# olofson/audiality2

Measured on AMD Instinct MI355X. Metric: voice-samples/sec + max realtime voices @48kHz, higher is better.
Workload: dtype int32; 1 GPU; 65536 voices 2xwtosc->panmix, 256 per group voice inline->fbdelay->fbdelay (benchmark/fmtest4.a2s delay settings; 256 groups, 512 fbdelays), 48 kHz, fragment=64, stereo (BASELINE configs[3]); voices_per_gpu=65536, chain=osc2-pan, groups=256

## Files before the change

### audiality2_amd/build.py

```python
import hashlib
import os
import shutil
import subprocess

HERE = os.path.dirname(os.path.abspath(__file__))
ROOT = os.path.dirname(HERE)
HIPCC = shutil.which("hipcc") or "/opt/rocm/bin/hipcc"


MARK = b"A2AMD_SRCHASH:"


def source_hash(sources, cmd=()):
    h = hashlib.sha256()
    for s in sources:
        h.update(os.path.basename(s).encode() + b"\0")
        with open(s, "rb") as f:
            h.update(f.read())
        h.update(b"\0")
    h.update(" ".join(cmd).encode())
    return h.hexdigest()[:32]


def stamped_hash(lib, mark=MARK):
    if not os.path.exists(lib):
        return None
    with open(lib, "rb") as f:
        blob = f.read()
    i = blob.find(mark)
    if i < 0:
        return None
    return blob[i + len(mark):i + len(mark) + 32].decode("ascii", "replace")


ENGMARK = b"A2AMD_ENGHASH:"


def engine_hash(engine):
    files = []
    for d in ("include", "src", os.path.join("src", "units"), os.path.join("src", "drivers")):
        p = os.path.join(engine, d)
        if os.path.isdir(p):
            files += [os.path.join(p, f) for f in sorted(os.listdir(p)) if f.endswith((".h", ".h.cmake", ".h.in"))]
    return source_hash(files, (stamped_hash(os.path.join(HERE, "liba2amd_units.so")) or "",))


def _stale(target, want):
    return stamped_hash(target) != want


def _define(h):
    return '-DA2AMD_SRCHASH="%s"' % h


def build_lib(force=False):
    csrc = os.path.join(HERE, "csrc")
    srcs = [os.path.join(csrc, f) for f in ("a2amd_host.cpp", "a2amd_sched.cpp", "a2amd_render.cpp", "a2amd_dist.cpp",
                                            "a2amd_vm.cpp", "a2amd_kernels.hip", "a2amd_fast.hip", "a2amd_vm.hip", "a2amd_wavecap.hip", "a2amd_wavepost.hip", "a2amd_win.hip", "a2amd_vmwin.hip", "a2amd_noise.hip", "a2amd_noisepan.hip", "a2amd_noisefiltpan.hip", "a2amd_cutsweep.hip", "a2amd_oscbare.hip")]
    deps = srcs + [os.path.join(csrc, "a2amd_host.h"), os.path.join(csrc, "a2amd_switches.h"), os.path.join(csrc, "a2amd_device.h"), os.path.join(csrc, "a2amd_dsp.h"),
                   os.path.join(csrc, "a2amd_fm.h"), os.path.join(csrc, "a2amd_vmcore.h"), os.path.join(csrc, "a2amd_taps.h"), os.path.join(csrc, "a2amd_winctl.h"), os.path.join(csrc, "a2amd_vmdev.h"), os.path.join(csrc, "a2amd_noisemap.h"), os.path.join(csrc, "a2amd_noisevoice.h"), os.path.join(csrc, "a2amd_settled.h"), os.path.join(csrc, "a2amd_cutsweep.h"), os.path.join(csrc, "a2amd_filt.h"), os.path.join(ROOT, "include", "a2amd.h"),
                   os.path.join(ROOT, "include", "a2amd_noise.h"), os.path.join(ROOT, "include", "a2amd_noisepan.h"), os.path.join(ROOT, "include", "a2amd_noisefilt.h"), os.path.join(ROOT, "include", "a2amd_sweep.h"), os.path.join(ROOT, "include", "a2amd_wavepost.h"),
                   os.path.join(ROOT, "include", "a2amd_bus.h"), os.path.join(ROOT, "include", "a2amd_oscbare.h"), os.path.join(ROOT, "include", "a2amd_fbdpan.h"), os.path.join(ROOT, "include", "a2amd_buswin.h"), os.path.join(ROOT, "include", "a2amd_vmbatch.h"), os.path.join(ROOT, "include", "a2amd_vm.h")]
    out = os.path.join(HERE, "liba2amd.so")
    flags = ["--offload-arch=gfx950", "-O3", "-std=c++17", "-fPIC", "-shared", "-Wno-unused-value"]
    want = source_hash(deps, flags)
    if force or _stale(out, want):
        subprocess.run([HIPCC] + flags + [_define(want), "-o", out] + srcs, check=True)
    return out


def build_units(force=False):
    src = os.path.join(HERE, "csrc", "a2amd_units.c")
    deps = [src, os.path.join(ROOT, "include", "a2amd.h"), os.path.join(ROOT, "include", "a2amd_noise.h"), os.path.join(ROOT, "include", "a2amd_noisepan.h"),
            os.path.join(ROOT, "include", "a2amd_noisefilt.h"), os.path.join(ROOT, "include", "a2amd_sweep.h"), os.path.join(ROOT, "include", "a2amd_bus.h"),
            os.path.join(ROOT, "include", "a2amd_wavepost.h"), os.path.join(ROOT, "include", "a2amd_oscbare.h"), os.path.join(ROOT, "include", "a2amd_fbdpan.h"), os.path.join(ROOT, "include", "a2amd_buswin.h"), os.path.join(ROOT, "include", "a2amd_vmbatch.h"), os.path.join(ROOT, "include", "a2amd_plugin.h"),
            os.path.join(ROOT, "include", "a2amd_walk.h"), os.path.join(ROOT, "include", "a2amd_vm.h")]
    out = os.path.join(HERE, "liba2amd_units.so")
    flags = ["-O2", "-Wall", "-fPIC", "-shared"]
    want = source_hash(deps, flags)
    if force or _stale(out, want):
        subprocess.run(["gcc"] + flags + [_define(want), "-o", out, src,
                        "-L" + HERE, "-la2amd", "-ldl", "-lpthread", "-lm", "-Wl,-rpath,$ORIGIN"], check=True)
    return out


def build_walk(force=False, engine=None):
    engine = engine or os.environ.get("A2_ENGINE_SRC", "/root/reference")
    out = os.path.join(HERE, "liba2amd_walk.so")
    src = os.path.join(HERE, "csrc", "a2amd_walk.c")
    own = [src, os.path.join(ROOT, "include", "a2amd_walk.h"), os.path.join(ROOT, "include", "a2amd_vm.h"),
           os.path.join(ROOT, "include", "a2amd_plugin.h")]
    flags = ["-O2", "-Wall", "-fPIC", "-shared"]
    want = source_hash(own, flags)
    kept = os.path.join(ROOT, "oracle", "_ref", "liba2amd_walk.so")
    if not (os.path.exists(os.path.join(engine, "src", "internals.h")) and shutil.which("cmake")):
        if (not os.path.exists(out) or _stale(out, want)) and not _stale(kept, want):
            shutil.copyfile(kept, out)
        if os.path.exists(out) and _stale(out, want):
            raise RuntimeError(f"{out} was not built from this tree's a2amd_walk.c (stamp {stamped_hash(out)}, "
                               f"sources {want}) and the engine's source tree ({engine}) is not here to rebuild it")
        return out if os.path.exists(out) else None
    inc = os.path.join(HERE, "_engine_include")
    weng = engine_hash(engine)
    if force or _stale(out, want) or stamped_hash(out, ENGMARK) != weng:
        subprocess.run(["cmake", f"-DENGINE={engine}", f"-DOUT={inc}", "-P", os.path.join(HERE, "csrc", "engine_header.cmake")],
                       check=True, stdout=subprocess.DEVNULL)
        subprocess.run(["gcc"] + flags + [_define(want), '-DA2AMD_ENGHASH="%s"' % weng, "-I" + inc] +
                       ["-I" + os.path.join(engine, d) for d in ("include", "src", "src/units", "src/drivers")] +
                       ["-o", out, src, "-L" + HERE, "-la2amd_units", "-la2amd", "-ldl", "-lpthread", "-Wl,-rpath,$ORIGIN"],
                       check=True)
    if stamped_hash(kept) != want or stamped_hash(kept, ENGMARK) != weng:
        os.makedirs(os.path.dirname(kept), exist_ok=True)
        shutil.copyfile(out, kept)
    return out


def build_oracle(force=False):
    odir = os.path.join(ROOT, "oracle")
    targets = ["restate"]
    if os.path.exists("/root/reference/src/core.c") and shutil.which("cmake"):
        targets += ["ref", "tools", "optionb"]
    subprocess.run(["make", "-s", "-C", odir] + (["-B"] if force else []) + targets, check=True)
    return os.path.join(odir, "liba2oracle.so")


def build_all(force=False):
    lib = build_lib(force)
    build_units(force)
    build_walk(force)
    return lib, build_oracle(force)
```

### audiality2_amd/csrc/a2amd_device.h

```cpp
#pragma once
#include <stdint.h>

#define A2D_MAXCHAIN   16
#define A2D_CHAIN_INLINE 8
#define A2D_MAXBATCH 256
#define FBW_MAXWIN (2 * A2D_MAXBATCH)
#define A2D_USTATE    24
#define A2D_MAXCH      8
#define A2D_FRAG      64
#define A2D_MIPS      10
#define A2D_FBD_BUFSIZE 131072
#define A2D_MAXPHINC  512
#define A2D_COEF_WORDS 3
#define A2D_WTOSC_MAXLENGTH (0x01000000 - 1 - 131)

enum { A2D_WTOSC = 0, A2D_PANMIX, A2D_FILTER12, A2D_FBDELAY, A2D_INLINE, A2D_XINSERT,
	A2D_FM1, A2D_FM2, A2D_FM3, A2D_FM4, A2D_FM3P, A2D_FM4P, A2D_FM2R, A2D_FM4R,
	A2D_DC, A2D_WAVESHAPER, A2D_DCBLOCK, A2D_LIMITER, A2D_XSINK, A2D_XSOURCE };
#define A2D_IS_FM(k) ((k) >= A2D_FM1 && (k) <= A2D_FM4R)

enum { A2D_OSC_OFF = 0, A2D_OSC_NOISE, A2D_OSC_WAVE, A2D_OSC_MIPWAVE };

#define A2D_DESC(kind, add, nin, nout, wired) \
	(((uint32_t)(kind) << 24) | ((uint32_t)(add) << 4) | ((uint32_t)(nin) << 8) | \
	 ((uint32_t)(nout) << 12) | ((uint32_t)(wired) << 16))
#define A2D_KIND(d)  ((d) >> 24)
#define A2D_ADD(d)   (((d) >> 4) & 1u)
#define A2D_NIN(d)   (((d) >> 8) & 15u)
#define A2D_NOUT(d)  (((d) >> 12) & 15u)
#define A2D_WIRED(d) (((d) >> 16) & 1u)

enum {
	OW_MODE = 0, OW_WAVE, OW_DPHASE, OW_PHASE_LO, OW_PHASE_HI, OW_NOISE,
	OW_PRAMPING, OW_P = 7, OW_A = 11, OW_SEED = 15 };
enum {
	PW_VOL = 0, PW_PAN = 4 };
enum {
	FW_Q = 0, FW_LP = 4, FW_BP, FW_HP, FW_F1, FW_D1A, FW_D1B, FW_D2A, FW_D2B,
	FW_F1NEXT, FW_RAMP };
enum {
	DW_FBDELAY = 0, DW_LDELAY, DW_RDELAY, DW_DRYGAIN, DW_FBGAIN, DW_LGAIN,
	DW_RGAIN, DW_BUFPOS, DW_BUFIDX };

enum {
	CW_VALUE = 0, CW_MODE = 4 };
enum {
	SW_AMOUNT = 0 };
enum {
	BW_F1 = 0, BW_D1A, BW_D1B, BW_D2A, BW_D2B };
enum {
	LW_RELEASE = 0, LW_THRESHOLD, LW_PEAK };
enum {
	MW_SLOT = 0 };
enum {
	FO_A = 0, FO_FB = 4, FO_P = 8, FO_LASTPITCH = 12, FO_PHASE, FO_DPHASE, FO_LAST, FO_WORDS };
#define A2D_FMSTATE 64

#define A2D_WF_RAWTAPS 0x40000000u

struct A2DWave {
	int32_t  type;
	uint32_t flags;
	uint32_t period;
	uint32_t size[A2D_MIPS];
	uint32_t off[A2D_MIPS];
	uint32_t pad;
};

struct A2DVoice {
	int32_t nunits;
	int32_t unit[A2D_CHAIN_INLINE];
	int32_t out_off, out_nch;
	int32_t own_off, own_nch;
	int32_t pad[3];
};

static_assert(sizeof(A2DVoice) == 64, "the voice record is one 64-byte line");
struct A2DVoiceExt { int32_t unit[A2D_MAXCHAIN - A2D_CHAIN_INLINE]; };

struct A2DRec {
	uint32_t head;
	int32_t  value;
	uint32_t dur;
	uint32_t start;
};
enum { R_SEG = 1, R_WRITE, R_INIT, R_KILL, R_F1SET, R_F1RAMP, R_NOISESEED, R_NOP };
#define A2D_HEAD(frag, op, unit, reg) \
	((uint32_t)(frag) | ((uint32_t)(op) << 16) | ((uint32_t)(unit) << 24) | ((uint32_t)(reg) << 28))
#define A2D_RFRAG(h) ((h) & 0xffffu)
#define A2D_ROP(h)   (((h) >> 16) & 0xffu)
#define A2D_RUNIT(h) (((h) >> 24) & 15u)
#define A2D_RREG(h)  (((h) >> 28) & 15u)

struct A2DRun { int32_t first, count; };

#define A2D_VM_NOWRITE 0xffu
#define A2D_VM_TRAPWRITE 0xfeu
#define A2D_VM_MAXCUT  2
#define A2D_VM_MAXENV  2
#define A2D_VM_MAXPOS  8
#define A2D_VM_ENVPOS  14
#define A2D_ENV_LUTSHIFT 6
#define A2D_ENV_LUTSIZE  (1 << A2D_ENV_LUTSHIFT)
#define A2D_ENV_LUTS     8
struct A2DVmEnv {
	int32_t ramper[4];
	int32_t lut;
	int32_t scale, offset, out;
	int32_t active;
	uint8_t regbase;
	uint8_t k;
	uint8_t target;
	uint8_t pad;
};
struct A2DVmVoice {
	uint32_t waketime;
	uint32_t code, ncode;
	uint16_t pc;
	uint8_t  state, ncut;
	int32_t  voice;
	int32_t  fault;
	uint8_t  cmap[64];
	uint8_t  kind[A2D_MAXCHAIN];
	uint8_t  cutpos[A2D_VM_MAXCUT];
	uint8_t  pad[2];
	int32_t  cut[A2D_VM_MAXCUT][4];
	A2DVmEnv env[A2D_VM_MAXENV];
	int32_t  nenv;
	uint32_t exit_when;
	int32_t  has_exit;
	int32_t  r[64];
};

struct A2DVmParams {
	A2DVmVoice     *vmv;
	const int      *list;
	int32_t         n;
	const uint32_t *code;
	const uint32_t *ptab;
	const int32_t  *f1tab;
	const uint16_t *envlut;
	A2DRun         *runs;
	A2DRun         *vmrun;
	A2DRec         *recs;
	uint32_t        rec_base, rec_cap;
	uint32_t       *total;
	uint32_t        now;
	uint32_t        msdur;
	int32_t         samplerate, basepitch;
	int32_t         nfrags;
	uint8_t         fragframes[A2D_MAXBATCH];
	uint8_t         fragbase[A2D_MAXBATCH];
};

enum { XW_SLOT = 0, XW_MODE = 1 };
#define A2D_XIO_HALF ((size_t)A2D_MAXBATCH * 8 * A2D_FRAG)
#define A2D_XIO_SLOT (2 * A2D_XIO_HALF)

#define A2D_FAST_FCH 8
#define A2D_OSC2_FCH 4
#define A2D_MAXVPW   32

struct A2DParams {
	const A2DVoice *voices;
	const A2DVoiceExt *vext;
	const uint32_t *udesc;
	int32_t        *ustate;
	int32_t        *vactive;
	const A2DRun   *runs;
	const A2DRec   *recs;
	const A2DWave  *waves;
	const int16_t  *wavepool;
	const int32_t  *wavecoef;
	int32_t        *busmem;
	int32_t        *fbdmem;
	const uint32_t *ptab;
	int32_t        *fmstate;
	const uint32_t *fmsine;
	int32_t *xio;
	const uint32_t *nseed;
	const int32_t  *nslot;
	int32_t         nnoise;
	const int32_t  *cutf;
	const int32_t  *cslot;
	int32_t         ncut;
	int32_t         nfrags;
	int32_t         samplerate;
	int32_t         debug;
	uint8_t         fragframes[A2D_MAXBATCH];
	uint16_t        fragstart[A2D_MAXBATCH];
};

#ifdef __HIPCC__
static inline __host__ __device__ bool a2d_noise_seed(const A2DParams &p, int f, int ui, unsigned *seed)
{
	if(!p.nseed)
		return false;
	const int k = p.nslot[ui];
	if(k <= 0 || k > p.nnoise)
		return false;
	*seed = p.nseed[(size_t)f * (size_t)p.nnoise + (size_t)(k - 1)];
	return true;
}
#endif

#ifdef __HIPCC__
static inline __host__ __device__ bool a2d_cut_coeff(const A2DParams &p, int f, int ui, int *f1)
{
	if(p.ncut <= 0)
		return false;
#if defined(__HIP_DEVICE_COMPILE__)
	typedef const __attribute__((address_space(4))) A2DParams *CP;
	typedef const __attribute__((address_space(4))) int32_t *CI;
	uintptr_t qa = (uintptr_t)&p;
	asm volatile("" : "+s"(qa));
	const CP q = (CP)qa;
	const int ncut = q->ncut;
	const int k = *((CI)(uintptr_t)q->cslot + ui);
	if(k <= 0 || k > ncut)
		return false;
	const int v = *((CI)(uintptr_t)q->cutf + ((size_t)f * (size_t)ncut + (size_t)(k - 1)));
#else
	const int k = p.cslot[ui];
	if(k <= 0 || k > p.ncut)
		return false;
	const int v = p.cutf[(size_t)f * (size_t)p.ncut + (size_t)(k - 1)];
#endif
	if(v < 0)
		return false;
	*f1 = v;
	return true;
}
#endif

struct A2DCutSweep { int32_t ramper[4]; int32_t unit, slot, pad[2]; };
int a2d_launch_cut_sweep(const A2DCutSweep *list, int n, int f0, int count, unsigned frames, int32_t *cutf, int stride,
		size_t words, int32_t *cslot, int nunits, void *stream);
int a2d_launch_cut_resolve(int32_t *cutf, size_t words, const int32_t *f1tab, void *stream);

struct A2DNoiseOsc { uint32_t ph_lo, ph_hi, dphase; int32_t unit, slot, pad[3]; };
int a2d_launch_noise_seeds(const A2DNoiseOsc *osc, int n, uint32_t start, int f0, int count, unsigned frames,
		uint32_t *seed, int stride, size_t seed_words, int32_t *nslot, int nunits, void *stream);

int a2d_launch_leaf_noisepan(const A2DParams *dparams, const A2DParams &hp, const int *dlist, int nlist, int vpw, void *stream);
int a2d_launch_leaf_noisefiltpan(const A2DParams *dparams, const A2DParams &hp, const int *dlist, int nlist, int vpg, void *stream);
int a2d_launch_leaf_oscbare(const A2DParams *dparams, const A2DParams &hp, const int *dlist, int nlist, int vpw, void *stream);

int a2d_launch_vm(const A2DVmParams &vp, int emit, void *stream);
int a2d_launch_vm_pool(const A2DVmParams &vp, unsigned *out, void *stream);
#define A2D_WIN_STAGED 2
struct A2DVmwOut {
	A2DVmVoice *vmv;
	int        *ustate;
	int        *vactive;
	A2DRun     *runs;
	uint32_t   *total;
	uint32_t   *idle;
};
int a2d_launch_vm_commit(const A2DVmParams &vp, const A2DParams &hp, int nosc, int filt, const A2DVmwOut &from, void *stream);
int a2d_launch_vm_win(const A2DVmParams &vp, const A2DParams &hp, int nosc, int filt, int fa, int fb, uint32_t now_fa,
		uint32_t batch_end, int *wslot, int *wext, int *wscr, unsigned *widx, unsigned *wtop, unsigned wcap, void *stream,
		const A2DVmwOut *out = nullptr);
#define A2D_VMW_ROW (64 - 1 - 1)

int a2d_launch_voices(const A2DParams *dparams, const int *dlist, int nlist, int vpw, void *stream);
enum { A2D_STAGED_NONE = 0, A2D_STAGED_PHASES, A2D_STAGED_FULL };
struct A2DCommit { const int *list; int nlist, nosc; const int *ustage; const unsigned char *staged; };
struct A2DCommitSet { A2DCommit c[2]; int n; };
int a2d_launch_leaf_oscpan(const A2DParams *dparams, const A2DParams &hp, const int *dlist, int nlist,
		int vpw, int ysplit, int *ustage, unsigned char *staged, void *stream, void *event_after_main, A2DCommit *defer);
int a2d_launch_bus_driver(const A2DParams *dparams, const int *dlist, int nlist, int nfrags, int consume,
		const A2DCommitSet *commits, void *stream, int *master_host = nullptr, int ramping = 0);
int a2d_launch_commit(const A2DParams &hp, const A2DCommit &cm, void *stream);
int a2d_launch_bus_fbdchain(const A2DParams *dparams, const int *dlist, int nlist, int consume, void *stream);
int a2d_launch_bus_fbdpan(const A2DParams *dparams, const int *dlist, int nlist, int consume, void *stream, int windows = 0);
int a2d_launch_park(int32_t *stage, int32_t *bus, unsigned words, void *stream);
int a2d_launch_add_bus(int32_t *dst, int32_t *src, unsigned words, void *stream);
int a2d_launch_add_inject(const int32_t *inj, int32_t *bus, int nch, int n, int nfrags, void *stream);
int a2d_launch_build_coef(const int16_t *pool, int *coef, unsigned lo, unsigned hi, void *stream);
int a2d_launch_capture(const int32_t *bus, int32_t *dst, const uint32_t *fragpos, int nfrags, int nch, void *stream);
int a2d_launch_wave_from_pcm(const int32_t *pcm, int16_t *pool, const uint32_t *off, const uint32_t *size, int levels, int looped,
		int pre, int post, void *stream);
int a2d_launch_wave_level0(const int32_t *pcm, int16_t *d, unsigned size, void *stream);
int a2d_launch_wave_finish(int16_t *pool, const uint32_t *off, const uint32_t *size, int levels, int looped, int pre, int post,
		void *stream);
unsigned a2d_wavepost_scratch_words(unsigned size, unsigned flags, unsigned chunk);
int a2d_launch_wave_level0_post(const int32_t *pcm, int16_t *d, unsigned size, unsigned flags, unsigned chunk, uint32_t *scratch,
		void *stream);
int a2d_osc2filtpan_max_vpg(void);
int a2d_launch_leaf_osc2filtpan(const A2DParams *dparams, const A2DParams &hp, const int *dlist, int nlist,
		int vpg, void *stream);
int a2d_launch_leaf_oscfiltpan(const A2DParams *dparams, const A2DParams &hp, const int *dlist, int nlist,
		int vpw, void *stream);
int a2d_launch_scatter_runs(const int *didx, const A2DRun *dval, int n, A2DRun *druns, void *stream);
int a2d_launch_leaf_osc2pan(const A2DParams *dparams, const A2DParams &hp, const int *dlist, int nlist,
		int vpw, int ysplit, int *ustage, unsigned char *staged, void *stream, A2DCommit *defer);
struct A2Switches;
int a2d_launch_leaf_recs(const A2Switches &sw, const A2DParams *dparams, const A2DParams &hp, int nosc, int filt, const int *dlist,
		int nlist, int vpw, void *stream, int skip_empty = 0);
#define A2D_WIN_WORDS 24
#define A2D_WIN_SLOTWORDS(nosc, filt) ((filt) ? ((nosc) == 1 ? 20 : 24) : ((nosc) == 1 ? 12 : 20))
int a2d_launch_win_ctl(const A2DParams *dparams, const A2DParams &hp, int nosc, int filt, const int *dlist, int nlist,
		int skip_empty, int fa, int fb, int *wslot, int *wext, unsigned *widx, unsigned *wtop, unsigned wcap, int *wrc,
		void *stream);
int a2d_launch_win_render(const A2Switches &sw, const A2DParams &hp, int nosc, int filt, const int *dlist, int nlist, int fa, int fb,
		const int *wslot, const int *wext, const unsigned *widx, void *stream);
int a2d_launch_leaf_recs_all(const A2Switches &sw, const A2DParams *dparams, const A2DParams &hp, const int *const *lists, const int *counts,
		int vpw, void *stream, int skip_mask = 0);
int a2d_launch_leaf_fmpan(const A2DParams *dparams, const A2DParams &hp, int kind, const int *dlist, int nlist,
		int vpw, void *stream);
int a2d_launch_leaf_fmpan_all(const A2DParams *dparams, const A2DParams &hp, const int *dlist,
		const int *count8, int vpw, void *stream);
```

### audiality2_amd/csrc/a2amd_fast.hip

```cpp
#include <hip/hip_runtime.h>
#include <type_traits>
#include <algorithm>
#include <stdlib.h>
#include "a2amd_device.h"
#include "a2amd_switches.h"
#include "a2amd_dsp.h"
#include "a2amd_fm.h"
#include "a2amd_filt.h"

#include "a2amd_taps.h"

__global__ void k_build_coef(const int16_t *__restrict__ pool, int *__restrict__ coef, unsigned lo, unsigned hi)
{
	const unsigned j = lo + blockIdx.x * blockDim.x + threadIdx.x;
	if(j >= hi)
		return;
	const int dm = pool[j - 1], d0 = pool[j], d1 = pool[j + 1], d2 = pool[j + 2];
	const int c = (d1 - dm) >> 1;
	const int a = (3 * (d0 - d1) + d2 - dm) >> 1;
	const int b = dm - d0 + c - a;
	int *e = coef + A2D_COEF_WORDS * (size_t)j;
	e[0] = a;
	e[1] = b;
	e[2] = (int)(((unsigned)c << 16) | ((unsigned)d0 & 0xffffu));
// ... 398 lines not shown
					phs[j] = ph;
					ph += (uint64_t)dph * (unsigned)nfr[j];
				}
			}
			const unsigned ldph = lane_dph(lane, dph);
			const int cb = coef_base(doff);
			if((raw_mask >> v) & 1ull) {
				const int16_t *d = wavepool + doff;
#pragma unroll
				for(int h = 0; h < FAST_FCH; h += 4) {
					Quad16 qa[4], qb[4];
					unsigned pa[4], pb[4];
#pragma unroll
					for(int j = 0; j < 4; ++j) {
						pa[j] = tap_phase(phs[h + j], ldph);
						pb[j] = pa[j] + (dph16 >> 1);
						qa[j] = *(const Quad16 *)(d + (int)(pa[j] >> 8) - 1);
						qb[j] = *(const Quad16 *)(d + (int)(pb[j] >> 8) - 1);
					}
#pragma unroll
					for(int j = 0; j < 4; ++j) {
						int sm = inter_quads(qa[j], qb[j], pa[j], pb[j]);
						int x = mul64s(sm, amp, 17);
						x = (lane < nfr[h + j]) ? x : 0;
						acc0[h + j] = wadd(acc0[h + j], mul64s(x, v0, 24));
						acc1[h + j] = wadd(acc1[h + j], mul64s(x, v1, 24));
					}
				}
			} else
#pragma unroll
			for(int h = 0; h < FAST_FCH; h += 4) {
				Coef4 ka[4], kb[4];
				unsigned pa[4], pb[4];
#pragma unroll
				for(int j = 0; j < 4; ++j) {
					pa[j] = tap_phase(phs[h + j], ldph);
					asm("" : "+v"(pa[j]));
					pb[j] = pa[j] + (dph16 >> 1);
					ka[j] = coef_at(crs, cb, pa[j]);
					kb[j] = coef_at(crs, cb, pb[j]);
				}
#pragma unroll
				for(int j = 0; j < 4; ++j) {
					int sm = inter_coefs(ka[j], pa[j], kb[j], pb[j]);
					int x = mul64s(sm, amp, 17);
					x = (lane < nfr[h + j]) ? x : 0;
					acc0[h + j] = wadd(acc0[h + j], mul64s(x, v0, 24));
					acc1[h + j] = wadd(acc1[h + j], mul64s(x, v1, 24));
				}
			}
			if(last_slice && c == c_hi - 1) {
				const bool me = lane == v;
				const uint64_t endph = ph << (unsigned)rdl(dv[DV_MM], v);
				WRL(phlo_l, (int)(unsigned)endph);
				WRL(phhi_l, (int)(unsigned)(endph >> 32));
			}
		}
		flush_acc(busmem, cur_off, cur_nch, f0, nf, lane, dbg, acc0, acc1);
	}

	const unsigned long long todo_mask = unsettled_mask & __ballot(lane % nslices == slice);
	if(todo_mask) {
		for(int f0 = 0; f0 < nfrags; f0 += FAST_FCH) {
			const int nf = min((int)FAST_FCH, nfrags - f0);
			int acc0[FAST_FCH], acc1[FAST_FCH];
#pragma unroll
			for(int j = 0; j < FAST_FCH; ++j)
				acc0[j] = acc1[j] = 0;
			int cur_off = rdl(my_off, 0), cur_nch = rdl(my_nch, 0);
			for(int v = 0; v < nv; ++v) {
				if(!((todo_mask >> v) & 1ull))
					continue;
				const int voff = rdl(my_off, v);
				if(voff != cur_off) {
					flush_acc(busmem, cur_off, cur_nch, f0, nf, lane, dbg, acc0, acc1);
					cur_off = voff;
					cur_nch = rdl(my_nch, v);
				}
				OscS o;
				Ramp vol, pan;
				const int *src = f0 ? ustage : ustate;
				osc_from_mem(o, src + (size_t)rdl(u0, v) * A2D_USTATE);
				{
					const volatile int *wpv = src + (size_t)rdl(u1, v) * A2D_USTATE;
					vol.value = rfl(wpv[0]); vol.target = rfl(wpv[1]); vol.delta = rfl(wpv[2]); vol.timer = rfl(wpv[3]);
					pan.value = rfl(wpv[4]); pan.target = rfl(wpv[5]); pan.delta = rfl(wpv[6]); pan.timer = rfl(wpv[7]);
				}
				for(int j = 0; j < nf; ++j) {
					int o0 = 0, o1 = 0;
					oscpan_fragment(g, o, vol, pan, frames_of(ffr, f0 + j), lane, o0, o1);
#pragma unroll
					for(int jj = 0; jj < FAST_FCH; ++jj)
						if(jj == j) {
							acc0[jj] = wadd(acc0[jj], o0);
							acc1[jj] = wadd(acc1[jj], o1);
						}
				}
				if(lane == 0) {
					osc_to_mem(ustage + (size_t)rdl(u0, v) * A2D_USTATE, o);
					int *wpv = ustage + (size_t)rdl(u1, v) * A2D_USTATE;
					wpv[0] = vol.value; wpv[1] = vol.target; wpv[2] = vol.delta; wpv[3] = vol.timer;
					wpv[4] = pan.value; wpv[5] = pan.target; wpv[6] = pan.delta; wpv[7] = pan.timer;
				}
			}
			flush_acc(busmem, cur_off, cur_nch, f0, nf, lane, dbg, acc0, acc1);
			__builtin_amdgcn_fence(__ATOMIC_RELEASE, "wavefront");
			__builtin_amdgcn_s_waitcnt(0);
		}
	}

	if(mine && dv[DV_SETTLED] && last_slice) {
		int *w0 = ustage + (size_t)u0 * A2D_USTATE;
		w0[OW_PHASE_LO] = phlo_l;
		w0[OW_PHASE_HI] = phhi_l;
	}
	if(ustage != ustate && lane < nv)
		stage_mark(staged + first + lane, mine, dv[DV_SETTLED] != 0, last_slice, lane % nslices == slice);
}

DEV void commit_block(const A2DCommit &cm, int block, const A2DVoice *__restrict__ voices, int *__restrict__ ustate)
{
	const int i = block * 256 + threadIdx.x;
	if(i >= cm.nlist * cm.nosc)
		return;
	const int e = i / cm.nosc, o = i - e * cm.nosc;
	const int what = cm.staged[e];
	if(what == A2D_STAGED_NONE)
		return;
	const A2DVoice &vc = voices[cm.list[e]];
	const size_t a = (size_t)vc.unit[o] * A2D_USTATE;
	ustate[a + OW_PHASE_LO] = cm.ustage[a + OW_PHASE_LO];
	ustate[a + OW_PHASE_HI] = cm.ustage[a + OW_PHASE_HI];
	if(what != A2D_STAGED_FULL)
		return;
	for(int k = 0; k < 15; ++k)
		if(k != OW_NOISE && k != OW_PHASE_LO && k != OW_PHASE_HI)
			ustate[a + k] = cm.ustage[a + k];
	if(o == 0) {
		const size_t ap = (size_t)vc.unit[cm.nosc] * A2D_USTATE;
		for(int k = 0; k < 8; ++k)
			ustate[ap + k] = cm.ustage[ap + k];
	}
}

DEV int commit_blocks(const A2DCommit &cm) { return (cm.nlist * cm.nosc + 255) / 256; }

__global__ __launch_bounds__(256)
void k_commit_oscpan(A2DCommit cm, const A2DVoice *__restrict__ voices, int *__restrict__ ustate)
{
	commit_block(cm, blockIdx.x, voices, ustate);
}

#define OSC2_FCH A2D_OSC2_FCH
enum { OV_MODE = 0, OV_WAVE, OV_DPHASE, OV_PHLO, OV_PHHI, OV_PRAMP, OV_P = 6, OV_A = 10, OV_NWORDS = 14 };
enum { OD_MM = 0, OD_DPH, OD_SIZEM, OD_DOFF, OD_NWORDS };

DEV void osc_from_lanes(OscS &o, const int (&so)[OV_NWORDS], int v)
{
	o.mode = rdl(so[OV_MODE], v);
	o.wave = rdl(so[OV_WAVE], v);
	o.dphase = (unsigned)rdl(so[OV_DPHASE], v);
	o.phase = (uint64_t)(unsigned)rdl(so[OV_PHLO], v) | ((uint64_t)(unsigned)rdl(so[OV_PHHI], v) << 32);
	o.p_ramping = rdl(so[OV_PRAMP], v);
	o.p.value = rdl(so[OV_P], v); o.p.target = rdl(so[OV_P + 1], v);
	o.p.delta = rdl(so[OV_P + 2], v); o.p.timer = rdl(so[OV_P + 3], v);
	o.a.value = rdl(so[OV_A], v); o.a.target = rdl(so[OV_A + 1], v);
	o.a.delta = rdl(so[OV_A + 2], v); o.a.timer = rdl(so[OV_A + 3], v);
	o.noise = 0;
	o.seed = 0;
}

DEV void osc_to_lanes(int (&so)[OV_NWORDS], const OscS &o, bool me)
{
	WRL(so[OV_MODE], o.mode);
	WRL(so[OV_WAVE], o.wave);
	WRL(so[OV_DPHASE], (int)o.dphase);
	WRL(so[OV_PHLO], (int)(unsigned)o.phase);
	WRL(so[OV_PHHI], (int)(unsigned)(o.phase >> 32));
	WRL(so[OV_PRAMP], o.p_ramping);
	WRL(so[OV_P], o.p.value); WRL(so[OV_P + 1], o.p.target);
	WRL(so[OV_P + 2], o.p.delta); WRL(so[OV_P + 3], o.p.timer);
	WRL(so[OV_A], o.a.value); WRL(so[OV_A + 1], o.a.target);
	WRL(so[OV_A + 2], o.a.delta); WRL(so[OV_A + 3], o.a.timer);
}

#define OSC2_WPE 4
__global__ __launch_bounds__(64 * FAST_WPB) __attribute__((amdgpu_waves_per_eu(OSC2_WPE, OSC2_WPE)))
void k_leaf_osc2pan(const A2DParams *__restrict__ pp, const int *__restrict__ list, int nlist, int vpw,
		int ysplit, const A2DVoice *__restrict__ voices, const int *ustate, int *ustage,
		const int16_t *__restrict__ wavepool, const A2DWave *__restrict__ waves,
		const uint32_t *__restrict__ ptab, int *__restrict__ busmem, const int *__restrict__ wavecoef,
		unsigned char *__restrict__ staged)
{
	const A2DParams &p = *pp;
	const int wv = rfl((int)(threadIdx.x >> 6));
	const int lane = threadIdx.x & 63;
	const int first = (blockIdx.x * FAST_WPB + wv) * vpw;
	if(first >= nlist)
		return;
	const int nv = min(vpw, nlist - first);
	const int nfrags = p.nfrags;
	const int dbg = p.debug;
	FastPtrs g = { wavepool, waves, ptab, dbg };
	const CoefRsrc crs = coef_rsrc(wavecoef);

	const int nchunks = (nfrags + OSC2_FCH - 1) / OSC2_FCH;
	const int per = (nchunks + ysplit - 1) / ysplit;
	const int slice = blockIdx.y;
	const int c_lo = slice * per, c_hi = min(nchunks, c_lo + per);
	const bool last_slice = c_hi >= nchunks;
	if(c_lo >= nchunks)
		return;
	const int nslices = (nchunks + per - 1) / per;

	int ffr[A2D_MAXBATCH / 64], fst[A2D_MAXBATCH / 64];
#pragma unroll
	for(int k = 0; k < A2D_MAXBATCH / 64; ++k) {
		ffr[k] = (k * 64 + lane < nfrags) ? p.fragframes[k * 64 + lane] : 0;
		fst[k] = (k * 64 + lane < nfrags) ? p.fragstart[k * 64 + lane] : 0;
	}

	int od[2][OD_NWORDS], amp_l[2] = { 0, 0 }, phlo_l[2] = { 0, 0 }, phhi_l[2] = { 0, 0 };
	int v0l = 0, v1l = 0, settled_l = 0;
	int uu[3] = { 0, 0, 0 }, my_off = -1, my_nch = 2;
	bool mine = false;
#pragma unroll
	for(int o = 0; o < 2; ++o)
#pragma unroll
		for(int k = 0; k < OD_NWORDS; ++k)
			od[o][k] = 0;
	if(lane < nv)
		mine = p.runs[list[first + lane]].count == 0;
	if(mine) {
		const A2DVoice &vc = voices[list[first + lane]];
		my_off = vc.out_off;
		my_nch = vc.out_nch;
		bool settled = true;
		int wave_l[2], dphase_l[2];
#pragma unroll
		for(int o = 0; o < 2; ++o) {
			uu[o] = vc.unit[o];
			const int *w = ustate + (size_t)uu[o] * A2D_USTATE;
			wave_l[o] = w[OW_WAVE];
			dphase_l[o] = w[OW_DPHASE];
			amp_l[o] = w[OW_A];
			phlo_l[o] = w[OW_PHASE_LO];
			phhi_l[o] = w[OW_PHASE_HI];
			settled = settled && a2s_osc_settled(w[OW_MODE], (unsigned)dphase_l[o], w[OW_PRAMPING], w + OW_P, w + OW_A);
		}
		uu[2] = vc.unit[2];
		const int *wp = ustate + (size_t)uu[2] * A2D_USTATE;
		int sp[8];
#pragma unroll
		for(int k = 0; k < 8; ++k)
			sp[k] = wp[k];
		settled = settled && a2s_arrived(sp + PW_VOL, sp + PW_PAN);
		if(settled) {
#pragma unroll
			for(int o = 0; o < 2; ++o)
				settled = settled_wave(waves + wave_l[o], (unsigned)dphase_l[o], od[o], settled);
			a2s_pan_gains(sp[PW_VOL], sp[PW_PAN], a2s_pan_over(sp[PW_PAN]), &v0l, &v1l);
		}
		settled_l = settled ? 1 : 0;
	}
	const unsigned long long unsettled_mask = __ballot(mine && !settled_l);

	for(int c = c_lo; c < c_hi; ++c) {
		const int f0 = c * OSC2_FCH;
		const int nf = min((int)OSC2_FCH, nfrags - f0);
		int acc0[OSC2_FCH], acc1[OSC2_FCH], nfr[OSC2_FCH];
#pragma unroll
		for(int j = 0; j < OSC2_FCH; ++j) {
			acc0[j] = acc1[j] = 0;
			nfr[j] = (j < nf) ? frames_of(ffr, f0 + j) : 0;
		}
		const unsigned before = (unsigned)frames_of(fst, f0);
		unsigned pre[OSC2_FCH];
		pre[0] = 0;
#pragma unroll
		for(int j = 1; j < OSC2_FCH; ++j)
			pre[j] = pre[j - 1] + (unsigned)nfr[j - 1];
		int cur_off = rdl(my_off, 0), cur_nch = rdl(my_nch, 0);
		for(int v = 0; v < nv; ++v) {
			if(!rdl(settled_l, v))
				continue;
			const int voff = rdl(my_off, v);
			if(voff != cur_off) {
				flush_acc(busmem, cur_off, cur_nch, f0, nf, lane, dbg, acc0, acc1);
				cur_off = voff;
				cur_nch = rdl(my_nch, v);
			}
			const int v0 = rdl(v0l, v), v1 = rdl(v1l, v);
			int xs[OSC2_FCH];
			uint64_t endph[2];
			Coef4 ka[2][OSC2_FCH], kb[2][OSC2_FCH];
			unsigned pa[2][OSC2_FCH], pb[2][OSC2_FCH];
			int amps[2];
#pragma unroll
			for(int o = 0; o < 2; ++o) {
				const unsigned mm = (unsigned)rdl(od[o][OD_MM], v), dph = (unsigned)rdl(od[o][OD_DPH], v);
				const unsigned sizem = (unsigned)rdl(od[o][OD_SIZEM], v), doff = (unsigned)rdl(od[o][OD_DOFF], v);
				amps[o] = rdl(amp_l[o], v);
				const uint64_t phase = (uint64_t)(unsigned)rdl(phlo_l[o], v) |
						((uint64_t)(unsigned)rdl(phhi_l[o], v) << 32);
				uint64_t ph = (phase >> mm) + (uint64_t)before * dph;
				const unsigned ldph = lane_dph(lane, dph);
				const int cb = coef_base(doff);
				uint64_t phs[OSC2_FCH];
				if(!(sizem & (sizem - 1)) && !(ph >> 48)) {
					const uint64_t mask = ((uint64_t)sizem << 24) - 1;
#pragma unroll
					for(int j = 0; j < OSC2_FCH; ++j)
						phs[j] = (ph + (uint64_t)dph * pre[j]) & mask;
					ph = phs[OSC2_FCH - 1] + (uint64_t)dph * (unsigned)nfr[OSC2_FCH - 1];
				} else {
#pragma unroll
					for(int j = 0; j < OSC2_FCH; ++j) {
						ph = wrap_phase(ph, sizem);
						phs[j] = ph;
						ph += (uint64_t)dph * (unsigned)nfr[j];
					}
				}
#pragma unroll
				for(int j = 0; j < OSC2_FCH; ++j) {
					pa[o][j] = tap_phase(phs[j], ldph);
					asm("" : "+v"(pa[o][j]));
					pb[o][j] = pa[o][j] + (dph >> 17);
					ka[o][j] = coef_at(crs, cb, pa[o][j]);
					kb[o][j] = coef_at(crs, cb, pb[o][j]);
				}
				endph[o] = ph << mm;
			}
#pragma unroll
			for(int o = 0; o < 2; ++o)
#pragma unroll
				for(int j = 0; j < OSC2_FCH; ++j) {
					const int y = mul64s(inter_coefs(ka[o][j], pa[o][j], kb[o][j], pb[o][j]), amps[o], 17);
					xs[j] = o ? wadd(xs[j], y) : y;
				}
#pragma unroll
			for(int j = 0; j < OSC2_FCH; ++j) {
				const int x = (lane < nfr[j]) ? xs[j] : 0;
				acc0[j] = wadd(acc0[j], mul64s(x, v0, 24));
				acc1[j] = wadd(acc1[j], mul64s(x, v1, 24));
			}
			if(last_slice && c == c_hi - 1) {
				const bool me = lane == v;
#pragma unroll
				for(int o = 0; o < 2; ++o) {
					WRL(phlo_l[o], (int)(unsigned)endph[o]);
					WRL(phhi_l[o], (int)(unsigned)(endph[o] >> 32));
				}
			}
		}
		flush_acc(busmem, cur_off, cur_nch, f0, nf, lane, dbg, acc0, acc1);
	}

	const unsigned long long todo_mask = unsettled_mask & __ballot(lane % nslices == slice);
	if(todo_mask) {
		for(int f0 = 0; f0 < nfrags; f0 += OSC2_FCH) {
			const int nf = min((int)OSC2_FCH, nfrags - f0);
			int acc0[OSC2_FCH], acc1[OSC2_FCH];
#pragma unroll
			for(int j = 0; j < OSC2_FCH; ++j)
				acc0[j] = acc1[j] = 0;
			int cur_off = rdl(my_off, 0), cur_nch = rdl(my_nch, 0);
			for(int v = 0; v < nv; ++v) {
				if(!((todo_mask >> v) & 1ull))
					continue;
				const int voff = rdl(my_off, v);
				if(voff != cur_off) {
					flush_acc(busmem, cur_off, cur_nch, f0, nf, lane, dbg, acc0, acc1);
					cur_off = voff;
					cur_nch = rdl(my_nch, v);
				}
				OscS oa, ob;
				Ramp vol, pan;
				const int *src = f0 ? ustage : ustate;
				osc_from_mem(oa, src + (size_t)rdl(uu[0], v) * A2D_USTATE);
				osc_from_mem(ob, src + (size_t)rdl(uu[1], v) * A2D_USTATE);
				{
					const volatile int *wpv = src + (size_t)rdl(uu[2], v) * A2D_USTATE;
					vol.value = rfl(wpv[0]); vol.target = rfl(wpv[1]); vol.delta = rfl(wpv[2]); vol.timer = rfl(wpv[3]);
					pan.value = rfl(wpv[4]); pan.target = rfl(wpv[5]); pan.delta = rfl(wpv[6]); pan.timer = rfl(wpv[7]);
				}
				for(int j = 0; j < nf; ++j) {
					const int n = frames_of(ffr, f0 + j);
					int o0 = 0, o1 = 0;
					const OscPend pa_ = osc_fragment_begin(g, oa, n, lane), pb_ = osc_fragment_begin(g, ob, n, lane);
					const int x = wadd(osc_fragment_end(pa_), osc_fragment_end(pb_));
					pan_fragment_s(vol, pan, x, n, lane, o0, o1);
#pragma unroll
					for(int jj = 0; jj < OSC2_FCH; ++jj)
						if(jj == j) {
							acc0[jj] = wadd(acc0[jj], o0);
							acc1[jj] = wadd(acc1[jj], o1);
						}
				}
				if(lane == 0) {
					osc_to_mem(ustage + (size_t)rdl(uu[0], v) * A2D_USTATE, oa);
					osc_to_mem(ustage + (size_t)rdl(uu[1], v) * A2D_USTATE, ob);
					int *wpv = ustage + (size_t)rdl(uu[2], v) * A2D_USTATE;
					wpv[0] = vol.value; wpv[1] = vol.target; wpv[2] = vol.delta; wpv[3] = vol.timer;
					wpv[4] = pan.value; wpv[5] = pan.target; wpv[6] = pan.delta; wpv[7] = pan.timer;
				}
			}
			flush_acc(busmem, cur_off, cur_nch, f0, nf, lane, dbg, acc0, acc1);
			__builtin_amdgcn_fence(__ATOMIC_RELEASE, "wavefront");
			__builtin_amdgcn_s_waitcnt(0);
		}
	}

	if(mine && settled_l && last_slice) {
#pragma unroll
		for(int o = 0; o < 2; ++o) {
			int *w = ustage + (size_t)uu[o] * A2D_USTATE;
			w[OW_PHASE_LO] = phlo_l[o];
			w[OW_PHASE_HI] = phhi_l[o];
		}
	}
	if(ustage != ustate && lane < nv)
		stage_mark(staged + first + lane, mine, settled_l != 0, last_slice, lane % nslices == slice);
}

#define RECS_FCH 4
#define RECS_WPB 8

DEV void osc_init_s(const FastPtrs &g, OscS &o, int pitch)
{
	o.wave = -1;
	o.mode = A2D_OSC_OFF;
	o.phase = 0;
	o.p_ramping = 0;
	o.noise = 0;
	o.seed = 0;
	ramp_init(o.a, 0);
	ramp_init(o.p, pitch);
	o.dphase = (unsigned)rfl((int)p2i(g.ptab, o.p.value >> 8));
}

DEV void osc_write_s(const FastPtrs &g, OscS &o, int reg, int v, int start, int dur)
{
	switch(reg) {
	  case 0: {
		int wt = 0;
		o.wave = v;
		if(v >= 0) {
			const A2DWave *w = g.waves + v;
			wt = w->type;
			if(wt == 3 && w->size[0] > (unsigned)A2D_WTOSC_MAXLENGTH)
				wt = 0;
		}
		if(wt == 3)
			o.mode = A2D_OSC_MIPWAVE;
		else if(wt == 1)
			o.mode = A2D_OSC_NOISE;
		else {
			o.wave = -1;
			o.mode = A2D_OSC_OFF;
		}
		break;
	  }
	  case 1:
		ramp_set(o.p, v, start, dur);
		if(!dur)
			o.p_ramping = 1;
		break;
	  case 2:
		ramp_set(o.a, v, start, dur);
		break;
	  case 3:
		if(o.wave < 0)
			o.phase = 0;
		else {
			const unsigned period = g.waves[o.wave].period;
			const int ph = (int)((unsigned)v + ((((unsigned)start) * (o.dphase >> 8)) >> 8));
			o.phase = (uint64_t)(((int64_t)ph * (int64_t)period) * 256);
		}
		break;
	}
}

enum { FS_Q = 0, FS_LP = 4, FS_BP, FS_HP, FS_F1, FS_D1, FS_D2, FS_F1NEXT, FS_RAMP, FS_NWORDS };
struct FiltS { Ramp q; int lp, bp, hp, f1, d1, d2, f1next, ramp; };

extern "C" __device__ int a2d_writelane(int src, int lane, int old) __asm("llvm.amdgcn.writelane.i32");
DEV int writelane_s(int y, int val, int sel)
{
	return a2d_writelane(val, sel, y);
}

#define F12_JSTEP \
	"s_nop 1\n\t" \
	"v_mov_b32_dpp %[bsh], %[B] wave_shr:1 row_mask:0xf bank_mask:0xf\n\t" \
	"v_ashrrev_i32 %[ds], 4, %[bsh]\n\t" \
	"v_mul_lo_u32 %[t1], %[F], %[ds]\n\t" \
	"v_ashrrev_i32 %[t1], 8, %[t1]\n\t" \
	"v_mul_lo_u32 %[t2], %[Q], %[ds]\n\t" \
	"v_ashrrev_i32 %[t2], 8, %[t2]\n\t" \
	"v_add_u32_dpp %[L], %[L], %[t1] wave_shr:1 row_mask:0xf bank_mask:0xf\n\t" \
	"v_sub_u32 %[H], %[X], %[L]\n\t" \
	"v_sub_u32 %[H], %[H], %[t2]\n\t" \
	"v_ashrrev_i32 %[t1], 4, %[H]\n\t" \
	"v_mul_lo_u32 %[t1], %[F], %[t1]\n\t" \
	"v_ashrrev_i32 %[t1], 8, %[t1]\n\t" \
	"v_add_u32 %[B], %[t1], %[bsh]\n\t"
DEV int filt_window_j(FiltS &fs, int x, int off, int len, int lane)
{
// ... 1640 lines not shown
#pragma unroll
	for(int k = 0; k < FBC_MAXD; ++k)
		if(k < nd) {
			const int *w = p.ustate + (size_t)vc.unit[k + 1] * A2D_USTATE;
			d[k].fb = rfl(w[DW_FBDELAY]); d[k].l = rfl(w[DW_LDELAY]); d[k].r = rfl(w[DW_RDELAY]);
			d[k].dry = rfl(w[DW_DRYGAIN]); d[k].fbg = rfl(w[DW_FBGAIN]); d[k].lg = rfl(w[DW_LGAIN]); d[k].rg = rfl(w[DW_RGAIN]);
			d[k].pos = rfl(w[DW_BUFPOS]);
			d[k].b0 = p.fbdmem + (size_t)rfl(w[DW_BUFIDX]) * 2 * A2D_FBD_BUFSIZE;
			d[k].b1 = d[k].b0 + A2D_FBD_BUFSIZE;
			d[k].add = rfl((int)A2D_ADD(p.udesc[vc.unit[k + 1]]));
			dmin = min(dmin, min(d[k].fb, min(d[k].l, d[k].r)));
			dmax = max(dmax, max(d[k].fb, max(d[k].l, d[k].r)));
		}
	__syncthreads();
	const bool rest = at_rest != 0;
	int rv0 = 0, rv1 = 0;
	if(rest) {
		const int vk = fr[0][0], vp = mul64s(fr[0][2], vk, 24);
		rv0 = wsub(vk, vp); rv1 = wadd(vk, vp);
		if(fr[0][4]) {
			const int lim = wshl(vk, 1);
			if(rv0 > lim) rv0 = lim;
			if(rv1 > lim) rv1 = lim;
		}
	}
	const int rf = max(1, min(dmin, A2D_FBD_BUFSIZE - dmax) / A2D_FRAG);
	int *own = p.busmem + vc.own_off;
	int *out = p.busmem + vc.out_off;
	const int out_nch = vc.out_nch;
	for(int f0 = 0; f0 < nfrags; f0 += rf) {
		const int fend = min(nfrags, f0 + rf);
		for(int idx = f0 * A2D_FRAG + (int)threadIdx.x; idx < fend * A2D_FRAG; idx += FBC_THREADS) {
			const int f = idx >> 6, lane = idx & 63;
			if(lane >= p.fragframes[f])
				continue;
			const int t = (int)p.fragstart[f] + lane;
			int *src = own + (size_t)f * 2 * A2D_FRAG;
			int x0 = src[lane], x1 = src[A2D_FRAG + lane];
			if(consume) {
				src[lane] = 0;
				src[A2D_FRAG + lane] = 0;
			}
#pragma unroll
			for(int k = 0; k < FBC_MAXD; ++k)
				if(k < nd) {
					const FbdU &u = d[k];
					const int pos = wadd(u.pos, t);
					int o0 = mul64s(u.b1[(pos - u.fb) & M], u.fbg, 16);
					int o1 = mul64s(u.b0[(pos - u.fb) & M], u.fbg, 16);
					const int t0 = u.b0[(pos - u.l) & M], t1 = u.b1[(pos - u.r) & M];
					u.b0[pos & M] = wadd(x0, o0);
					u.b1[pos & M] = wadd(x1, o1);
					o0 = wadd(o0, mul64s(t0, u.lg, 16));
					o1 = wadd(o1, mul64s(t1, u.rg, 16));
					o0 = wadd(o0, mul64s(x0, u.dry, 16));
					o1 = wadd(o1, mul64s(x1, u.dry, 16));
					if(u.add) {
						x0 = wadd(x0, o0);
						x1 = wadd(x1, o1);
					} else {
						x0 = o0;
						x1 = o1;
					}
				}
			int v0 = rv0, v1 = rv1;
			if(!rest) {
				int r = f, wk = lane;
				if constexpr(WIN) {
					r = min((int)wfirst[f], FBW_MAXWIN - 1);
					const int rl = min((int)wfirst[f + 1], FBW_MAXWIN) - 1;
					while(r < rl && lane >= (fr[r][4] >> 16))
						++r;
					wk = lane - ((fr[r][4] >> 8) & 0xff);
				}
				const int vk = wadd(fr[r][0], wmul(fr[r][1], wk));
				const int pk = wadd(fr[r][2], wmul(fr[r][3], wk));
				const int vp = mul64s(pk, vk, 24);
				v0 = wsub(vk, vp); v1 = wadd(vk, vp);
				if(WIN ? fr[r][4] & 1 : fr[r][4]) {
					const int lim = wshl(vk, 1);
					if(v0 > lim) v0 = lim;
					if(v1 > lim) v1 = lim;
				}
			}
			const int o0 = mul64s(x0, v0, 24), o1 = mul64s(x1, v1, 24);
			int *dst = out + (size_t)f * out_nch * A2D_FRAG;
			if(o0)
				atomicAdd(&dst[lane], o0);
			if(o1)
				atomicAdd(&dst[A2D_FRAG + lane], o1);
		}
		if(fend < nfrags)
			__syncthreads();
	}
	if(threadIdx.x == 0) {
		int total = 0;
		for(int f = 0; f < nfrags; ++f)
			total += p.fragframes[f];
#pragma unroll
		for(int k = 0; k < FBC_MAXD; ++k)
			if(k < nd)
				p.ustate[(size_t)vc.unit[k + 1] * A2D_USTATE + DW_BUFPOS] = wadd(d[k].pos, total);
	}
}

__global__ __launch_bounds__(FBC_THREADS)
void k_bus_fbdpan(const A2DParams *__restrict__ pp, const int *__restrict__ list, int nlist, int consume)
{
	bus_fbdpan<false>(pp, list, consume);
}

__global__ __launch_bounds__(FBC_THREADS)
void k_bus_fbdpan_win(const A2DParams *__restrict__ pp, const int *__restrict__ list, int nlist, int consume)
{
	bus_fbdpan<true>(pp, list, consume);
}

int a2d_launch_bus_fbdpan(const A2DParams *dparams, const int *dlist, int nlist, int consume, void *stream, int windows)
{
	if(nlist <= 0)
		return 0;
	hipLaunchKernelGGL(windows ? k_bus_fbdpan_win : k_bus_fbdpan, dim3(nlist), dim3(FBC_THREADS), 0, (hipStream_t)stream,
			dparams, dlist, nlist, consume);
	return (int)hipGetLastError();
}

int a2d_launch_leaf_oscpan(const A2DParams *dparams, const A2DParams &hp, const int *dlist, int nlist,
		int vpw, int ysplit, int *ustage, unsigned char *staged, void *stream, void *event_after_main, A2DCommit *defer)
{
	if(nlist <= 0)
		return 0;
	vpw = vpw < 1 ? 1 : (vpw > 64 ? 64 : vpw);
	if(ysplit < 1 || !ustage || !staged)
		ysplit = 1;
	int nwaves = (nlist + vpw - 1) / vpw;
	int nblocks = (nwaves + FAST_WPB - 1) / FAST_WPB;
	hipLaunchKernelGGL(k_leaf_oscpan, dim3(nblocks, ysplit), dim3(64 * FAST_WPB), 0, (hipStream_t)stream,
			dparams, dlist, nlist, vpw, ysplit, hp.voices, (const int *)hp.ustate,
			ysplit > 1 ? ustage : hp.ustate, hp.wavepool, hp.waves, hp.ptab, hp.busmem, hp.wavecoef, staged);
	if(event_after_main)
		hipEventRecord((hipEvent_t)event_after_main, (hipStream_t)stream);
	if(ysplit > 1) {
		A2DCommit cm = { dlist, nlist, 1, ustage, staged };
		if(defer)
			*defer = cm;
		else
			a2d_launch_commit(hp, cm, stream);
	} else if(defer)
		defer->nlist = 0;
	return (int)hipGetLastError();
}

int a2d_launch_leaf_osc2pan(const A2DParams *dparams, const A2DParams &hp, const int *dlist, int nlist,
		int vpw, int ysplit, int *ustage, unsigned char *staged, void *stream, A2DCommit *defer)
{
	if(nlist <= 0)
		return 0;
	vpw = vpw < 1 ? 1 : (vpw > 64 ? 64 : vpw);
	if(ysplit < 1 || !ustage || !staged)
		ysplit = 1;
	int nwaves = (nlist + vpw - 1) / vpw;
	int nblocks = (nwaves + FAST_WPB - 1) / FAST_WPB;
	hipLaunchKernelGGL(k_leaf_osc2pan, dim3(nblocks, ysplit), dim3(64 * FAST_WPB), 0, (hipStream_t)stream,
			dparams, dlist, nlist, vpw, ysplit, hp.voices, (const int *)hp.ustate,
			ysplit > 1 ? ustage : hp.ustate, hp.wavepool, hp.waves, hp.ptab, hp.busmem, hp.wavecoef, staged);
	if(ysplit > 1) {
		A2DCommit cm = { dlist, nlist, 2, ustage, staged };
		if(defer)
			*defer = cm;
		else
			a2d_launch_commit(hp, cm, stream);
	} else if(defer)
		defer->nlist = 0;
	return (int)hipGetLastError();
}

__global__ void k_scatter_runs(const int *__restrict__ idx, const A2DRun *__restrict__ val, int n,
		A2DRun *__restrict__ runs)
{
	int i = blockIdx.x * blockDim.x + threadIdx.x;
	if(i < n)
		runs[idx[i]] = val[i];
}

int a2d_launch_scatter_runs(const int *didx, const A2DRun *dval, int n, A2DRun *druns, void *stream)
{
	if(n <= 0)
		return 0;
	hipLaunchKernelGGL(k_scatter_runs, dim3((n + 255) / 256), dim3(256), 0, (hipStream_t)stream,
			didx, dval, n, druns);
	return (int)hipGetLastError();
}

int a2d_launch_leaf_oscfiltpan(const A2DParams *dparams, const A2DParams &hp, const int *dlist, int nlist,
		int vpg, void *stream)
{
	if(nlist <= 0)
		return 0;
	vpg = vpg < 1 ? 1 : (vpg > FILT_MAXV ? FILT_MAXV : vpg);
	int nblocks = (nlist + vpg - 1) / vpg;
	size_t lds = (size_t)3 * vpg * FILT_PITCH * sizeof(int);
	hipLaunchKernelGGL(k_leaf_oscfiltpan, dim3(nblocks), dim3(64 * FILT_WAVES), lds, (hipStream_t)stream,
			dparams, dlist, nlist, vpg, hp.voices, hp.ustate, hp.wavepool, hp.waves, hp.ptab, hp.busmem, hp.wavecoef);
	return (int)hipGetLastError();
}

int a2d_osc2filtpan_max_vpg(void)
{
	const int nfull = FILT_WAVES - 1 - (FILT_WAVES / 4 - 1);
	const int v = nfull * (FILT2_LAUNCHV < FILT2_FASTV ? FILT2_LAUNCHV : FILT2_FASTV);
	return v > FILT_MAXV ? FILT_MAXV : v;
}

int a2d_launch_leaf_osc2filtpan(const A2DParams *dparams, const A2DParams &hp, const int *dlist, int nlist,
		int vpg, void *stream)
{
	if(nlist <= 0)
		return 0;
	vpg = vpg < 1 ? 1 : (vpg > FILT_MAXV ? FILT_MAXV : vpg);
	int nblocks = (nlist + vpg - 1) / vpg;
	size_t lds = (size_t)3 * vpg * FILT_PITCH * sizeof(int);
	hipLaunchKernelGGL(k_leaf_osc2filtpan, dim3(nblocks), dim3(64 * FILT_WAVES), lds, (hipStream_t)stream,
			dparams, dlist, nlist, vpg, hp.voices, hp.ustate, hp.wavepool, hp.waves, hp.ptab, hp.busmem, hp.wavecoef);
	return (int)hipGetLastError();
}

enum { PV_VOL = 0, PV_PAN = 4, PV_NWORDS = 8 };

DEV void pan_window_s(Ramp &vol, Ramp &pan, int x, int off, int len, int lane, int &acc0, int &acc1)
{
	const bool clamp = a2s_pan_over(pan.target) || a2s_pan_over(pan.value);
	ramp_prepare_s(vol, len);
	ramp_prepare_s(pan, len);
	const int k = lane - off;
	if(k >= 0 && k < len) {
		int vk = wadd(vol.value, wmul(vol.delta, k));
		int pk = wadd(pan.value, wmul(pan.delta, k));
		int vp = mul64s(pk, vk, 24);
		int v0 = wsub(vk, vp), v1 = wadd(vk, vp);
		if(clamp) {
			int lim = wshl(vk, 1);
			if(v0 > lim) v0 = lim;
			if(v1 > lim) v1 = lim;
		}
		acc0 = wadd(acc0, mul64s(x, v0, 24));
		acc1 = wadd(acc1, mul64s(x, v1, 24));
	}
	ramp_run(vol, len);
	ramp_run(pan, len);
}

template<int NOPS, int OSBITS, int PAR>
DEV void fmpan_body(const A2DParams &p, const int *__restrict__ list, int first, int nv, int lane,
		int *tile, const uint32_t *sine, const A2DVoice *__restrict__ voices, int *ustate,
		int *fmstate, const uint32_t *__restrict__ ptab, int *__restrict__ busmem)
{
	const int nfrags = p.nfrags;
	const int dbg = p.debug;
	const A2DRec *__restrict__ recs = p.recs;
	int ffr[A2D_MAXBATCH / 64];
#pragma unroll
	for(int k = 0; k < A2D_MAXBATCH / 64; ++k)
		ffr[k] = (k * 64 + lane < nfrags) ? p.fragframes[k * 64 + lane] : 0;

	int pv[PV_NWORDS];
#pragma unroll
	for(int k = 0; k < PV_NWORDS; ++k)
		pv[k] = 0;
	FmOp op[NOPS];
#pragma unroll
	for(int i = 0; i < NOPS; ++i) {
		op[i].a = op[i].fb = op[i].p = Ramp{ 0, 0, 0, 0 };
		op[i].last_pitch = op[i].last = 0;
		op[i].phase = op[i].dphase = 0;
	}
	unsigned step[NOPS], fix[NOPS];
#pragma unroll
	for(int i = 0; i < NOPS; ++i)
		step[i] = fix[i] = 0;
	int slot = -1, u0 = 0, u1 = 0, my_off = -1, my_nch = 2, v0 = 0, v1 = 0, settled = 0;
	int run_first = 0, run_count = 0, fmslot = -1;
	int actB = 0;
	const bool writer = lane < nv;
	if(lane < nv)
		slot = list[first + lane];
	else if(lane < 16 && !(p.debug & 4))
		slot = list[first + lane % nv];
	const bool mine = slot >= 0;
	const unsigned long long mine_mask = __ballot(mine);
	if(mine) {
		const A2DVoice &vc = voices[slot];
		u0 = vc.unit[0];
		u1 = vc.unit[1];
		my_off = vc.out_off;
		my_nch = vc.out_nch;
		const A2DRun run = p.runs[slot];
		run_first = run.first;
		run_count = run.count;
		actB = p.vactive[slot];
	}
	bool touched = mine && actB;
	if(touched) {
		fmslot = ustate[(size_t)u0 * A2D_USTATE + MW_SLOT];
		const int *fw = fmstate + (size_t)fmslot * A2D_FMSTATE;
#pragma unroll
		for(int i = 0; i < NOPS; ++i)
			fmop_load(op[i], fw + i * FO_WORDS);
		const int *w1 = ustate + (size_t)u1 * A2D_USTATE;
#pragma unroll
		for(int k = 0; k < 4; ++k) {
			pv[PV_VOL + k] = w1[PW_VOL + k];
			pv[PV_PAN + k] = w1[PW_PAN + k];
		}
		settled = !run_count && a2s_arrived(pv + PV_VOL, pv + PV_PAN);
		if(settled)
			a2s_pan_gains(pv[PV_VOL], pv[PV_PAN], a2s_pan_over(pv[PV_PAN]), &v0, &v1);
	}
	int curB = 0, curC = 0, actC = actB;
// ... 389 lines not shown
```

### audiality2_amd/csrc/a2amd_host.h

```cpp
#ifndef A2AMD_HOST_H
#define A2AMD_HOST_H
#include <hip/hip_runtime.h>
#include <rccl/rccl.h>
#include <dlfcn.h>
#include <math.h>
#include <stdarg.h>
#include <stdio.h>
#include <stdlib.h>
#include <string.h>
#include <algorithm>
#include <map>
#include <vector>
#include <future>

#include "../../include/a2amd.h"
#include "../../include/a2amd_vm.h"
#include "a2amd_device.h"
#include "a2amd_switches.h"

#ifndef M_PI
#define M_PI 3.14159265358979323846
#endif

namespace a2h {
// ... 231 lines not shown
	bool pred_valid = false;
	uint64_t pred_serial = 0;
	uint32_t pred_now = 0;
	uint32_t pred_span = 0;
	size_t pred_entries = 0;
	uint64_t pred_why[7] = { 0, 0, 0, 0, 0, 0, 0 };
	DevBuf<int> d_swin[2], d_swext[2], d_swscr;
	DevBuf<unsigned> d_swidx[2];
	int spec_set = 0;
	bool spec_launched_now = false;
	unsigned *d_swtop = nullptr;
	DevBuf<A2DVmVoice> d_vmv_sh;
	DevBuf<int> d_ustate_sh, d_vactive_sh;
	DevBuf<A2DRun> d_runs_sh;
	uint32_t *d_stotal = nullptr;
	unsigned *h_spec = nullptr;
	bool spec_valid = false;
	bool spec_use = false;
	int spec_nfrags = 0, spec_cls[3] = { 0, 0, 0 };
	uint8_t spec_ff[A2D_MAXBATCH], spec_fb[A2D_MAXBATCH];
	uint32_t cut_hint[16];
	int n_cut_hint = 0;
	size_t spec_cap = 0;
	size_t spec_demand = 0;
	uint64_t spec_launched = 0, spec_taken = 0, spec_overflows = 0;
	uint64_t spec_skip[4] = { 0, 0, 0, 0 }, spec_miss[4] = { 0, 0, 0, 0 };
	uint64_t spec_waits = 0;
	uint64_t rebuilt_at = 0;
	bool list_dirty = false;
	std::vector<std::pair<int, A2DVmVoice>> to_upload;
	uint32_t t0 = 0;
	bool t0_valid = false;
	uint32_t msdur = 0;
	uint64_t batch_time = 0;
	uint64_t replayed = 0;
	std::vector<int32_t> f1tab;
	std::future<std::vector<int32_t>> f1_future;
	uint32_t f1_future_sum = 0;
	uint32_t f1tab_sum = 0;
	bool f1tab_up = false;
	std::vector<A2DVmVoice> snap;
	std::vector<uint8_t> snap_have;
	int snap_fetches = 0;
	uint32_t rec_cap = 0;
	size_t rec_off = 0;
	a2amd_vm_stats stats = {};
	int unwalked = -1;
	DevBuf<A2DVmVoice> d_vmv;
	DevBuf<uint32_t> d_code;
	DevBuf<int> d_list;
	DevBuf<A2DRun> d_vmrun;
	int32_t *d_f1tab = nullptr;
	std::vector<uint16_t> envlut;
	uint16_t *d_envlut = nullptr;
	bool envlut_up = false;
	uint32_t *d_total = nullptr, *h_total = nullptr;
	uint32_t last_total = 0;
	a2amd_vm_batch_info last = {};
	A2DVmVoice *h_stage = nullptr;
	size_t h_stage_cap = 0;
};
}
using namespace a2h;

struct a2amd_ctx {
	a2amd_config cfg;
	char err[256];
	hipStream_t stream = nullptr;
	bool own_stream = false;
	hipEvent_t ev0 = nullptr, ev1 = nullptr, ev2 = nullptr;
	bool profiling = false;
	std::vector<hipEvent_t> ev_pool;
	size_t ev_used = 0;
	uint32_t ptab[128];

	std::vector<HUnit> units;
	std::vector<int> free_units, deferred_free_units;
	std::vector<HVoice> voices;
	std::vector<int> free_voices, deferred_free_voices;
	std::vector<HWave> waves;
	int building = -1;
	std::vector<int> stack;
	std::vector<A2DRec> up_recs;
	std::vector<int> up_idx, up_now;
	std::vector<A2DRun> up_val;
	std::vector<int> with_recs, prev_with_recs;
	std::vector<int> dirty_voices;
	long long serial_base = 0;
	bool o2f_quiet = true;
	int n_started_live = 0;
	int walked_started = 0;
	int n_noise = 0, n_cutoff_ramps = 0;
	std::vector<int> noise_order;
	long long noise_order_serial = -1, walk_serial = -2;
	struct NoiseStretch { int f0, count; unsigned frames; uint32_t start; size_t first, n; };
	std::vector<NoiseStretch> noise_st;
	std::vector<A2DNoiseOsc> noise_osc;
	int noise_slots = 0;
	DevBuf<uint32_t> d_nseed;
	DevBuf<int32_t> d_nslot;
	std::vector<int> sweeping;
	struct CutStretch { int f0, count; unsigned frames; size_t first, n; };
	std::vector<CutStretch> cut_st;
	std::vector<A2DCutSweep> cut_list;
	int cut_slots = 0;
	DevBuf<int32_t> d_cutf;
	DevBuf<int32_t> d_cslot;
	a2amd_sweep_batch_info last_sweeps = {};
	uint32_t n_cut_standin = 0;
	uint32_t n_cut_windows = 0;
	bool owners_all_driver = false;
	bool consume_ok = false;
	bool others_clean = false;
	bool root_clean = false;
	bool capturing = false;
	int n_clients = 0;
	int sub_resume = -1;
	int paused_at = 0;
	std::vector<int32_t> snap_ustate, snap_vactive;
	bool snap_valid = false;
	std::vector<uint8_t> defmap;
	bool defmap_used = false;
	bool defmap_dirty = false;
	std::vector<uint8_t> held;
	size_t n_held = 0;
	uint64_t walk_time = 0;
	unsigned prev_frames = 0;

	bool frag_open = false;
	int cur_frag = 0, nfrags = 0;
	unsigned fragframes[A2D_MAXBATCH];
	uint8_t fragbase[A2D_MAXBATCH];
	bool uploaded = false;

	std::vector<A2DVoice> mvoices;
	std::vector<A2DVoiceExt> mvext;
	bool long_chains = false;
	std::vector<uint32_t> mudesc;
	std::vector<A2DWave> mwaves;
	bool voices_dirty = true, udesc_dirty = true, waves_dirty = true, lists_dirty = true, ptab_dirty = true;
	std::vector<int> list_all;
	ListRange leaf[LEAF_N];
	int fm_kind_count[8] = { 0 };
	std::vector<DepthRange> depth_ranges;
	ListRange dyn[DYN_N];
	A2Switches sw;
	a2amd_batch_info last_batch = {};
	a2amd_noise_batch_info last_noise = {};
	uint32_t n_noise_standin = 0, n_noise_quiet = 0;
	uint32_t n_noise_filt_quiet = 0;
	a2amd_noise_filter_batch_info last_noise_filter = {};
	uint32_t n_bare_quiet = 0, n_bare_gliding = 0, n_bare_records = 0, n_mono_drivers = 0;
	a2amd_bare_batch_info last_bare = {};
	a2amd_fbdpan_batch_info last_fbdpan = {};
	a2amd_bus_windows_info last_buswin = {};
	a2amd_bus_info last_bus = {};
	uint32_t n_bus_windows_dropped = 0;

	size_t bus_stride_frames;
	size_t bus_used = 0;
	std::map<int, std::vector<int>> bus_free;
	std::vector<std::pair<int,int>> deferred_bus_free;

	int fbd_count = 0;
	std::vector<int> fbd_free, fbd_deferred_free, fbd_to_zero;
	int fm_count = 0;
	std::vector<int> fm_free, fm_deferred_free;

	std::vector<XioSlot> xio;
	std::vector<int> xio_free, xio_deferred_free;

	size_t wavepool_used = 0;
	std::vector<std::pair<size_t, size_t>> wavepool_free;
	std::vector<std::pair<size_t, size_t>> deferred_wavepool_free;
	std::vector<int> free_wave_slots, deferred_wave_slots;

	DevBuf<A2DVoice> d_voices;
	DevBuf<A2DVoiceExt> d_vext;
	DevBuf<uint32_t> d_udesc;
	DevBuf<int32_t> d_ustate;
	DevBuf<int32_t> d_ustage;
	DevBuf<int32_t> d_vactive;
	DevBuf<A2DRun> d_runs;
	DevBuf<A2DRec> d_recs;
	DevBuf<A2DWave> d_waves;
	DevBuf<int16_t> d_wavepool;
	DevBuf<int32_t> d_wavecoef;
	DevBuf<int32_t> d_busmem;
	DevBuf<int32_t> d_fbdmem;
	DevBuf<int32_t> d_fmstate;
	DevBuf<int32_t> d_xio;
	uint32_t *d_fmsine = nullptr;
	DevBuf<int> d_list;
	DevBuf<unsigned char> d_staged;
	DevBuf<int> d_scatter;
	uint32_t *d_ptab = nullptr;
	A2DParams *d_params = nullptr;
	DevBuf<char> d_blob;
	char *h_blob[2] = { nullptr, nullptr };
	size_t h_blob_cap[2] = { 0, 0 };
	hipEvent_t blob_ev[2] = { nullptr, nullptr };
	bool blob_busy[2] = { false, false };
	int blob_i = 0;
	const int *d_dyn = nullptr;
	A2DParams hparams;
	hipGraph_t graph[12] = {};
	hipGraphExec_t gexec[12] = {};
	const int32_t *gdst[12] = {};
	bool gdirect[12] = {};
	uint32_t gconsume[12] = {};
	struct Capture { int32_t *d = nullptr; size_t cap = 0, n = 0; bool on = false; uint32_t *d_fragpos = nullptr; } capture;
	DevBuf<uint32_t> d_wavepost;
	uint64_t wave_h2d_bytes = 0;
	uint32_t waves_uploaded = 0, waves_resident = 0;
	int32_t *master_dst = nullptr;
	bool master_direct = false;
	int32_t *h_master = nullptr;
	size_t h_master_cap = 0;
	bool blob_quiet = false;
	int blob_nfrags = 0;
	unsigned blob_frames[A2D_MAXBATCH];
	int quiet_streak = 0;
	struct Readback {
		int32_t *h = nullptr;
		size_t cap = 0;
		hipEvent_t ev = nullptr;
		int nfrags = 0;
		unsigned total = 0;
		uint8_t frames[A2D_MAXBATCH];
	} rb[2];
	int rb_head = 0, rb_count = 0;

	ncclComm_t comm = nullptr;
	int dist_rank = 0, dist_ranks = 1;
	bool dist_local = false;
	hipEvent_t grp_ev = nullptr;

	std::vector<int> moving;
	size_t n_moving_listed = 0;
	DevBuf<int> d_win, d_wext, d_wrc, d_wscr;
	DevBuf<unsigned> d_widx;
	unsigned *d_wtop = nullptr;
	unsigned *h_wtop = nullptr;
	hipEvent_t wtop_ev = nullptr;
	bool wtop_pending = false;
	hipStream_t win_fork[7] = { nullptr, nullptr, nullptr, nullptr, nullptr, nullptr, nullptr };
	hipEvent_t win_fev[8] = { nullptr, nullptr, nullptr, nullptr, nullptr, nullptr, nullptr, nullptr };
	hipStream_t win_stream = nullptr;
	hipEvent_t win_ev[5] = { nullptr, nullptr, nullptr, nullptr, nullptr };

	a2amd_stats stats;
	VmHost vm;

	int fail(int code, const char *fmt, ...)
	{
		va_list ap;
		va_start(ap, fmt);
		vsnprintf(err, sizeof(err), fmt, ap);
		va_end(ap);
		snprintf(g_err, sizeof(g_err), "%s", err);
		return code;
	}
};

static inline void use_device(const a2amd_ctx *c) { (void)hipSetDevice(c->cfg.device); }

namespace a2h {
template<class T>
int grow(a2amd_ctx *c, DevBuf<T> &b, size_t need, size_t elem_mult, bool keep)
{
	if(need <= b.cap)
		return 0;
	size_t ncap = std::max(need, b.cap ? b.cap * 2 : (elem_mult >= 65536 ? (size_t)2 : (size_t)1024));
	T *nd = nullptr;
	HIPCHK(c, hipMalloc((void **)&nd, ncap * elem_mult * sizeof(T)));
	if(keep && b.d && b.cap) {
		HIPCHK(c, hipStreamSynchronize(c->stream));
		HIPCHK(c, hipMemcpyAsync(nd, b.d, b.cap * elem_mult * sizeof(T), hipMemcpyDeviceToDevice, c->stream));
	}
	if(keep)
		HIPCHK(c, hipMemsetAsync((char *)nd + b.cap * elem_mult * sizeof(T), 0,
				(ncap - b.cap) * elem_mult * sizeof(T), c->stream));
	if(keep)
		HIPCHK(c, hipStreamSynchronize(c->stream));
	if(b.d) {
		HIPCHK(c, hipStreamSynchronize(c->stream));
		if(c->vm.pred_stream)
			HIPCHK(c, hipStreamSynchronize(c->vm.pred_stream));
		HIPCHK(c, hipFree(b.d));
	}
	b.d = nd;
	b.cap = ncap;
	return 0;
}

inline int rec_tag(const a2amd_ctx *c) { return c->frag_open ? c->cur_frag : c->nfrags; }
static inline bool is_held(const a2amd_ctx *c, int vi)
{
	return (size_t)vi < c->held.size() && c->held[vi];
}

static inline void unhold(a2amd_ctx *c, int vi)
{
	if(is_held(c, vi)) {
		c->held[vi] = 0;
		--c->n_held;
// ... 65 lines not shown
```

### audiality2_amd/csrc/a2amd_render.cpp

```cpp
#include "a2amd_host.h"

extern "C" {
static double now_us()
{
	timespec ts;
	clock_gettime(CLOCK_MONOTONIC, &ts);
	return ts.tv_sec * 1e6 + ts.tv_nsec * 1e-3;
}
static double g_t[4], g_n;
static double g_why[13];
static double g_cnt[6];
struct TimingDump { ~TimingDump() {
	A2Switches sw; a2amd_read_switches(&sw); if(sw.hosttiming && g_n) fprintf(stderr,
	"a2amd host timing per render: upload %.1f us, issue %.1f us, readback %.1f us (%g renders; %g quiet uploads, "
	"%g graph launches, %g records, %g voices with records, %g walk scans, %g R_NOPs)\n",
	g_t[0] / g_n, g_t[1] / g_n, g_t[2] / g_n, g_n, g_cnt[0], g_cnt[5], g_cnt[1], g_cnt[4], g_cnt[2], g_cnt[3]);
	if(sw.hosttiming && g_n) { fprintf(stderr, "a2amd uploads by first reason against the quiet path "
	"(blob, recs, prev recs, voices, udesc, waves, lists, ptab, dirty voices, fbd, nfrags, bus, none):");
	for(int k = 0; k < 13; ++k) fprintf(stderr, " %g", g_why[k]); fprintf(stderr, "\n"); } } } g_timing_dump;

}
namespace a2h { double *dbg_counters() { return g_cnt; } double *dbg_why() { return g_why; } }
extern "C" {

// ... 288 lines not shown
	unsigned pos = 0;
	for(int f = 0; f < rb.nfrags; ++f) {
		for(int ch = 0; ch < nch; ++ch)
			memcpy(out[ch] + pos, rb.h + ((size_t)f * nch + ch) * A2D_FRAG, rb.frames[f] * sizeof(int32_t));
		pos += rb.frames[f];
	}
	c->rb_head ^= 1;
	--c->rb_count;
	return (int)rb.total;
}

int a2amd_replay(a2amd_ctx *c, unsigned steps)
{
	use_device(c);
	c->snap_valid = false;
	const int GRAPH_STEPS = 8;
	if(!c->uploaded || !c->nfrags)
		return c->fail(A2AMD_ESTATE, "replay without an uploaded batch");
	if(!c->noise_st.empty())
		return c->fail(A2AMD_EUNSUPPORTED, "replay of a batch with device-seeded noise windows "
				"(a2amd_fragment_repeat_noise): a re-run would need a new generator word");
	if(!c->cut_st.empty())
		return c->fail(A2AMD_EUNSUPPORTED, "replay of a batch with a cutoff sweep table "
				"(a2amd_fragment_repeat with a sweeping filter): a re-run would need the ramp to go on");
	for(int vi = 0; vi < (int)c->voices.size(); ++vi)
		if(!c->voices[vi].recs.empty())
			return c->fail(A2AMD_ESTATE, "replay of a batch that carries command records");
	bool graphs = c->stream != nullptr && !c->profiling && !c->sw.no_graph && c->vm.list.empty();
	c->master_dst = nullptr;
	c->master_direct = false;
	if(graphs && (!c->gexec[0] || !c->gexec[1])) {
		if(build_graph(c, 0, GRAPH_STEPS) || build_graph(c, 1, 1)) {
			drop_graphs(c);
			graphs = false;
		}
	}
	while(steps) {
		if(graphs && steps >= (unsigned)GRAPH_STEPS) {
			if(int r = ensure_clean(c))
				return r;
			HIPCHK(c, hipGraphLaunch(c->gexec[0], c->stream));
			c->others_clean = c->root_clean = c->consume_ok;
			steps -= GRAPH_STEPS;
			c->stats.fragments += (uint64_t)c->nfrags * GRAPH_STEPS;
			c->stats.voice_fragments += (uint64_t)c->nfrags * c->list_all.size() * GRAPH_STEPS;
		} else if(graphs) {
			if(int r = ensure_clean(c))
				return r;
			HIPCHK(c, hipGraphLaunch(c->gexec[1], c->stream));
			c->others_clean = c->root_clean = c->consume_ok;
			--steps;
			c->stats.fragments += c->nfrags;
			c->stats.voice_fragments += (uint64_t)c->nfrags * c->list_all.size();
		} else {
			if(c->profiling) {
				if(c->ev_used + 3 > c->ev_pool.size())
					for(int i = 0; i < 3; ++i) {
						hipEvent_t e;
						HIPCHK(c, hipEventCreate(&e));
						c->ev_pool.push_back(e);
					}
				c->ev0 = c->ev_pool[c->ev_used];
				c->ev1 = c->ev_pool[c->ev_used + 1];
				c->ev2 = c->ev_pool[c->ev_used + 2];
				c->ev_used += 3;
			}
			if(int r = c->profiling ?
					issue_kernels(c, A2AMD_RENDER_SUBTREES | A2AMD_RENDER_ROOT, c->ev0, c->ev1, c->ev2) :
					issue_kernels(c, A2AMD_RENDER_SUBTREES | A2AMD_RENDER_ROOT, nullptr, nullptr, nullptr))
				return r;
			--steps;
		}
	}
	return A2AMD_OK;
}

static int drain_events(a2amd_ctx *c)
{
	if(!c->ev_used)
		return 0;
	HIPCHK(c, hipStreamSynchronize(c->stream));
	for(size_t i = 0; i + 2 < c->ev_used + 0 && i + 2 < c->ev_pool.size(); i += 3) {
		float a = 0, b = 0;
		if(hipEventElapsedTime(&a, c->ev_pool[i], c->ev_pool[i + 1]) == hipSuccess &&
				hipEventElapsedTime(&b, c->ev_pool[i], c->ev_pool[i + 2]) == hipSuccess) {
			c->stats.timed_leaf_ms += a;
			c->stats.timed_all_ms += b;
			++c->stats.timed_batches;
		}
	}
	c->ev_used = 0;
	return 0;
}

int a2amd_get_stats(a2amd_ctx *c, a2amd_stats *st)
{
	if(c->profiling)
		if(int r = drain_events(c))
			return r;
	*st = c->stats;
	return A2AMD_OK;
}

int a2amd_last_batch(const a2amd_ctx *c, a2amd_batch_info *bi)
{
	if(!c || !bi)
		return A2AMD_EINVAL;
	*bi = c->last_batch;
	return A2AMD_OK;
}

int a2amd_last_batch_noise(const a2amd_ctx *c, a2amd_noise_batch_info *out)
{
	if(!c || !out)
		return A2AMD_EINVAL;
	*out = c->last_noise;
	return A2AMD_OK;
}

int a2amd_last_batch_noise_filter(const a2amd_ctx *c, a2amd_noise_filter_batch_info *out)
{
	if(!c || !out)
		return A2AMD_EINVAL;
	*out = c->last_noise_filter;
	out->min_voices = (uint32_t)c->sw.nzf_min;
	return A2AMD_OK;
}

int a2amd_last_batch_sweeps(const a2amd_ctx *c, a2amd_sweep_batch_info *out)
{
	if(!c || !out)
		return A2AMD_EINVAL;
	*out = c->last_sweeps;
	return A2AMD_OK;
}

int a2amd_last_batch_buses(const a2amd_ctx *c, a2amd_bus_info *out)
{
	if(!c || !out)
		return A2AMD_EINVAL;
	*out = c->last_bus;
	out->master_direct = c->master_direct;
	return A2AMD_OK;
}

int a2amd_last_batch_bare(const a2amd_ctx *c, a2amd_bare_batch_info *out)
{
	if(!c || !out)
		return A2AMD_EINVAL;
	*out = c->last_bare;
	return A2AMD_OK;
}

int a2amd_last_batch_fbdpan(const a2amd_ctx *c, a2amd_fbdpan_batch_info *out)
{
	if(!c || !out)
		return A2AMD_EINVAL;
	*out = c->last_fbdpan;
	return A2AMD_OK;
}

int a2amd_last_batch_bus_windows(const a2amd_ctx *c, a2amd_bus_windows_info *out)
{
	if(!c || !out)
		return A2AMD_EINVAL;
	*out = c->last_buswin;
	out->window_cap = FBW_MAXWIN;
	return A2AMD_OK;
}

int a2amd_set_profiling(a2amd_ctx *c, int on)
{
	if(int r = drain_events(c))
		return r;
	if(on) {
		c->stats.timed_leaf_ms = c->stats.timed_all_ms = 0;
		c->stats.timed_batches = 0;
	}
	c->profiling = on != 0;
	return A2AMD_OK;
}

}
```

### audiality2_amd/csrc/a2amd_sched.cpp

```cpp
#include "a2amd_host.h"
#include "a2amd_cutsweep.h"
#include <functional>

namespace a2h {




void touch(a2amd_ctx *c, int vi)
{
	HVoice &v = c->voices[vi];
	const long long serial = c->serial_base + rec_tag(c);
	if(v.touched != serial) {
		v.touched = serial;
		v.frag_mark = v.recs.size();
	}
}



void spell_out_pending(a2amd_ctx *c, int vi)
{
	HVoice &dv = c->voices[vi];
	const bool marked = c->frag_open && c->defmap_used && (size_t)vi < c->defmap.size() && c->defmap[vi];
// ... 1369 lines not shown
			if(c->vm.spec_go_pending) {
				HIPCHK(c, hipStreamWaitEvent(c->stream, c->vm.spec_go, 0));
				c->vm.spec_go_pending = false;
			}
		}
		at = atw = 0;
		for(int j = 0; j < nj; ++j) {
			const Job &b = jobs[j];
			if(b.spec) {
				if(fa == 0 && a2d_launch_win_render(c->sw, c->hparams, b.nosc, b.filt, b.list, b.n, 0, nfrags, c->vm.d_swin[sset].d + b.satw,
						c->vm.d_swext[sset].d, c->vm.d_swidx[sset].d + b.sat, c->stream))
					return c->fail(A2AMD_EHIP, "window render launch failed: %s", hipGetErrorString(hipGetLastError()));
				if(fa == 0)
					++c->stats.launches;
				continue;
			}
			if(a2d_launch_win_render(c->sw, c->hparams, b.nosc, b.filt, b.list, b.n, fa, fb, wslot + atw,
					wext, widx + at, c->stream))
				return c->fail(A2AMD_EHIP, "window render launch failed: %s", hipGetErrorString(hipGetLastError()));
			at += (size_t)b.n * (size_t)(fb - fa);
			atw += (size_t)b.n * (size_t)(fb - fa) * A2D_WIN_SLOTWORDS(b.nosc, b.filt);
			++c->stats.launches;
		}
		if(two)
			HIPCHK(c, hipEventRecord(c->win_ev[2 + set], c->stream));
		if(wtiming && !two && !c->capturing) {
			float t_ctl = 0, t_ren = 0;
			HIPCHK(c, hipEventRecord(tev[2], c->stream));
			HIPCHK(c, hipEventSynchronize(tev[2]));
			hipEventElapsedTime(&t_ctl, tev[0], tev[1]);
			hipEventElapsedTime(&t_ren, tev[1], tev[2]);
			fprintf(stderr, "a2amd windows: fragments [%d, %d), %zu voices in %d list(s), %zu records: control pass %.1f us, render pass %.1f us\n",
					fa, fb, nvoices, nj, nrec, t_ctl * 1e3, t_ren * 1e3);
		}
	}
	if(!c->capturing && plain_jobs) {
		if(!c->h_wtop) {
			HIPCHK(c, hipHostMalloc((void **)&c->h_wtop, 4 * sizeof(unsigned), hipHostMallocDefault));
			memset(c->h_wtop, 0, 4 * sizeof(unsigned));
			HIPCHK(c, hipEventCreateWithFlags(&c->wtop_ev, hipEventDisableTiming));
		}
		HIPCHK(c, hipMemcpyAsync(c->h_wtop, c->d_wtop, 4 * sizeof(unsigned), hipMemcpyDeviceToHost, c->stream));
		HIPCHK(c, hipEventRecord(c->wtop_ev, c->stream));
		c->wtop_pending = true;
	}
	if(c->vm.fused && !c->vm.spec_use)
		if(int r = vm_fused_done(c))
			return r;
	if(c->sw.win_check && !c->capturing && plain_jobs) {
		unsigned top[4] = { 0, 0, 0, 0 };
		HIPCHK(c, hipMemcpyAsync(top, c->d_wtop, sizeof(top), hipMemcpyDeviceToHost, c->stream));
		HIPCHK(c, hipStreamSynchronize(c->stream));
		if(top[1] || (two && top[3])) {
			if(c->vm.fused)
				c->vm.fused_off = true;
			return c->fail(A2AMD_ESTATE, "window pool overflow (%u / %u of %zu entries)", top[0], top[2], c->d_wext.cap);
		}
	}
	return 0;
}

static void flush_commits(a2amd_ctx *c, A2DCommitSet *pend)
{
	for(int k = 0; k < pend->n; ++k)
		a2d_launch_commit(c->hparams, pend->c[k], c->stream);
	pend->n = 0;
}

static int launch_recs(a2amd_ctx *c, int nosc, int filt, const int *list, int n, int skip_empty)
{
	if(!n)
		return 0;
	const int vpw = c->sw.rvpw_set ? c->sw.rvpw : (n + 8191) / 8192;
	if(a2d_launch_leaf_recs(c->sw, c->d_params, c->hparams, nosc, filt, list, n, vpw, c->stream, skip_empty))
		return c->fail(A2AMD_EHIP, "leaf records launch failed: %s", hipGetErrorString(hipGetLastError()));
	++c->stats.launches;
	return 0;
}

static bool oscpan_alone(const a2amd_ctx *c)
{
	for(int k = 0; k < LEAF_N; ++k)
		if((c->leaf[k].count != 0) != (k == LEAF_OSCPAN))
			return false;
	return c->dyn[DYN_REST].first + c->dyn[DYN_REST].count == 0;
}

struct LeafPass {
	A2DCommitSet *pend;
	hipEvent_t e1;
	bool use_win;
	bool solo;
	bool done;
};

static int launch_leaves(a2amd_ctx *c, LeafPass &lp)
{
	if(lp.done)
		return 0;
	lp.done = true;
	A2DCommitSet &pend = *lp.pend;
	const int *const list = c->d_list.d;
	auto none_quiet = [&](int k, int nleaf) {
		return (c->sw.vmskip & (k == 2 ? 2 : 1)) && c->vm.spec_use && !c->vm.list.empty() && c->vm.n_cls[k] == nleaf && c->vm.spec_idle[k] == 0;
	};
	const ListRange oscpan = c->leaf[LEAF_OSCPAN];
	if(oscpan.count && none_quiet(0, oscpan.count)) {
		if(lp.solo && lp.e1)
			HIPCHK(c, hipEventRecord(lp.e1, c->stream));
		++c->vm.quiet_skipped;
	} else if(oscpan.count) {
		int vpw, ysplit;
		pick_fast_shape(c->sw, oscpan.count, c->nfrags, &vpw, &ysplit);
		if(a2d_launch_leaf_oscpan(c->d_params, c->hparams, list + oscpan.first, oscpan.count,
				vpw, ysplit, c->d_ustage.d, c->d_staged.d + oscpan.first, c->stream, lp.solo ? (void *)lp.e1 : nullptr,
				&pend.c[pend.n]))
			return c->fail(A2AMD_EHIP, "fast leaf launch failed: %s", hipGetErrorString(hipGetLastError()));
		if(pend.c[pend.n].nlist)
			++pend.n;
		++c->stats.launches;
		c->vm.last.quiet_launched[0] = 1;
	}
	const ListRange noisepan = c->leaf[LEAF_NOISEPAN];
	if(noisepan.count && !c->noise_st.empty() && c->n_noise_quiet) {
		const int vpw = c->sw.nzvpw_set ? c->sw.nzvpw : (noisepan.count + 1023) / 1024;
		if(a2d_launch_leaf_noisepan(c->d_params, c->hparams, list + noisepan.first, noisepan.count, vpw, c->stream))
			return c->fail(A2AMD_EHIP, "noise leaf launch failed: %s", hipGetErrorString(hipGetLastError()));
		++c->stats.launches;
		c->last_noise.quiet_launched = 1;
	}
	const ListRange noisefilt = c->leaf[LEAF_NOISEFILTPAN];
	if(noisefilt.count && !c->noise_st.empty() && c->n_noise_filt_quiet) {
		const int vpg = c->sw.nzfvpg_set ? c->sw.nzfvpg : (noisefilt.count + 255) / 256;
		if(a2d_launch_leaf_noisefiltpan(c->d_params, c->hparams, list + noisefilt.first, noisefilt.count, vpg, c->stream))
			return c->fail(A2AMD_EHIP, "noise filter leaf launch failed: %s", hipGetErrorString(hipGetLastError()));
		++c->stats.launches;
		c->last_noise_filter.quiet_launched = 1;
	}
	const ListRange bare = c->leaf[LEAF_OSCBARE];
	if(bare.count && c->n_bare_quiet) {
		const int vpw = std::min(std::max(c->sw.vpw_set ? c->sw.vpw : (bare.count + 1023) / 1024, 1), 64);
		if(a2d_launch_leaf_oscbare(c->d_params, c->hparams, list + bare.first, bare.count, vpw, c->stream))
			return c->fail(A2AMD_EHIP, "bare oscillator leaf launch failed: %s", hipGetErrorString(hipGetLastError()));
		++c->stats.launches;
		c->last_bare.launched = 1;
		c->last_bare.vpw = (uint32_t)vpw;
	}
	const ListRange osc2pan = c->leaf[LEAF_OSC2PAN];
	if(osc2pan.count && none_quiet(1, osc2pan.count))
		++c->vm.quiet_skipped;
	else if(osc2pan.count) {
		int vpw, ysplit;
		pick_fast_shape(c->sw, osc2pan.count, c->nfrags * A2D_FAST_FCH / A2D_OSC2_FCH, &vpw, &ysplit, 16);
		if(a2d_launch_leaf_osc2pan(c->d_params, c->hparams, list + osc2pan.first, osc2pan.count,
				vpw, ysplit, c->d_ustage.d, c->d_staged.d + osc2pan.first, c->stream, &pend.c[pend.n]))
			return c->fail(A2AMD_EHIP, "2-osc leaf launch failed: %s", hipGetErrorString(hipGetLastError()));
		if(pend.c[pend.n].nlist)
			++pend.n;
		++c->stats.launches;
		c->vm.last.quiet_launched[1] = 1;
	}
	const ListRange oscfilt = c->leaf[LEAF_OSCFILTPAN];
	if(oscfilt.count && none_quiet(2, oscfilt.count))
		++c->vm.quiet_skipped;
	else if(oscfilt.count) {
		const int nf = oscfilt.count;
		int vpw = c->sw.fvpw_set ? c->sw.fvpw : std::min(std::max((nf + 255) / 256, 1), 64);
		if(a2d_launch_leaf_oscfiltpan(c->d_params, c->hparams, list + oscfilt.first, nf, vpw, c->stream))
			return c->fail(A2AMD_EHIP, "filter leaf launch failed: %s", hipGetErrorString(hipGetLastError()));
		++c->stats.launches;
		c->vm.last.quiet_launched[2] = 1;
	}
	const ListRange o2f = c->leaf[LEAF_OSC2FILTPAN];
	if(o2f.count && c->o2f_quiet) {
		const int nf = o2f.count;
		const int maxv = a2d_osc2filtpan_max_vpg();
		const int rounds = std::max(1, (nf + 256 * maxv - 1) / (256 * maxv));
		const int vpg = c->sw.f2vpw ? c->sw.f2vpw : std::min(std::max((nf + 256 * rounds - 1) / (256 * rounds), 1), maxv);
		if(a2d_launch_leaf_osc2filtpan(c->d_params, c->hparams, list + o2f.first, nf, vpg, c->stream))
			return c->fail(A2AMD_EHIP, "2-osc filter leaf launch failed: %s", hipGetErrorString(hipGetLastError()));
		++c->stats.launches;
		c->last_batch.o2f_launched = 1;
		c->last_batch.o2f_voices = (uint32_t)nf;
		c->last_batch.o2f_max_vpg = (uint32_t)maxv;
		c->last_batch.o2f_vpg = (uint32_t)std::min(std::max(vpg, 1), 64);
	}
	const ListRange fm = c->leaf[LEAF_FMPAN];
	int fm_kinds = 0;
	for(int k = 0; k < 8; ++k)
		fm_kinds += c->fm_kind_count[k] != 0;
	if(fm_kinds > 1 && fm.count <= 16384 && !c->sw.fmvpw_set) {
		if(a2d_launch_leaf_fmpan_all(c->d_params, c->hparams, list + fm.first, c->fm_kind_count, (fm.count + 1023) / 1024, c->stream))
			return c->fail(A2AMD_EHIP, "fm leaf launch failed: %s", hipGetErrorString(hipGetLastError()));
		++c->stats.launches;
	} else {
		for(int k = 0, at = fm.first; k < 8; at += c->fm_kind_count[k++]) {
			const int n = c->fm_kind_count[k];
			if(!n)
				continue;
			int vpw = c->sw.fmvpw_set ? c->sw.fmvpw : (n + 1023) / 1024;
			vpw = std::min(std::max(vpw, 1), 64);
			if(a2d_launch_leaf_fmpan(c->d_params, c->hparams, A2AMD_FM1 + k, list + at, n, vpw, c->stream))
				return c->fail(A2AMD_EHIP, "fm leaf launch failed: %s", hipGetErrorString(hipGetLastError()));
			++c->stats.launches;
		}
	}
	const ListRange gen = c->leaf[LEAF_GENERIC];
	if(gen.count) {
		if(a2d_launch_voices(c->d_params, list + gen.first, gen.count, pick_vpw(gen.count), c->stream))
			return c->fail(A2AMD_EHIP, "leaf launch failed: %s", hipGetErrorString(hipGetLastError()));
		++c->stats.launches;
	}
	if(!lp.use_win) {
		static const int nosc[4] = { 1, 2, 1, 2 }, filt[4] = { 0, 0, 1, 1 };
		const int *lists[4];
		int counts[4], total = 0, kinds = 0;
		for(int k = 0; k < 4; ++k) {
			lists[k] = c->d_dyn + c->dyn[k].first;
			counts[k] = c->dyn[k].count;
			total += counts[k];
			kinds += counts[k] != 0;
		}
		c->last_batch.recs_voices = (uint32_t)total;
		if(!c->vm.list.empty())
			c->last_batch.recs_voices += (uint32_t)(c->vm.n_cls[0] + c->vm.n_cls[1] + c->vm.n_cls[2]);
		if(kinds > 1 && total <= 4096 && !c->sw.rvpw_set) {
			if(a2d_launch_leaf_recs_all(c->sw, c->d_params, c->hparams, lists, counts, 1, c->stream, c->o2f_quiet ? 8 : 0))
				return c->fail(A2AMD_EHIP, "leaf records launch failed: %s", hipGetErrorString(hipGetLastError()));
			++c->stats.launches;
		} else {
			for(int k = 0; k < 4; ++k)
				if(int r = launch_recs(c, nosc[k], filt[k], lists[k], counts[k], k == DYN_FILT2 && c->o2f_quiet))
					return r;
		}
		if(!c->vm.list.empty()) {
			const int *l = c->vm.d_list.d + c->vm.list.size();
			for(int k = 0; k < 3; l += c->vm.n_cls[k++])
				if(int r = launch_recs(c, nosc[k], filt[k], l, c->vm.n_cls[k], 1))
					return r;
		}
	}
	const ListRange rest = c->dyn[DYN_REST];
	if(rest.count > 0) {
		if(a2d_launch_voices(c->d_params, c->d_dyn + rest.first, rest.count, pick_vpw(rest.count), c->stream))
			return c->fail(A2AMD_EHIP, "leaf launch failed: %s", hipGetErrorString(hipGetLastError()));
		++c->stats.launches;
	}
	return 0;
}

static int issue_leaf_phase(a2amd_ctx *c, bool consume, bool consume_sub, hipEvent_t e0, hipEvent_t e1, A2DCommitSet *pend)
{
	const bool selfclean = consume || consume_sub;
	if(c->capturing ? !selfclean : !(selfclean && c->others_clean && c->root_clean))
		HIPCHK(c, hipMemsetAsync(c->d_busmem.d, 0, c->bus_used * sizeof(int32_t), c->stream));
	c->others_clean = selfclean;
	c->root_clean = consume;
	if(e0)
		HIPCHK(c, hipEventRecord(e0, c->stream));
	bool use_win;
	{
		int nwinv = 0;
		for(int k = DYN_OSC1; k <= DYN_FILT2; ++k)
			nwinv += c->dyn[k].count;
		for(int k = 0; k < 3; ++k)
			nwinv += c->vm.list.empty() ? 0 : c->vm.n_cls[k];
		use_win = c->sw.win >= 0 ? c->sw.win != 0 : nwinv >= c->sw.win_min;
	}
	const bool vmwin_ok = c->sw.vmwin;
	if(int r = vm_issue(c, use_win && vmwin_ok && !c->vm.fused_off))
		return r;
	c->last_batch = a2amd_batch_info{};
	c->last_batch.o2f_class = (uint32_t)c->leaf[LEAF_OSC2FILTPAN].count;
	c->last_batch.o2f_listed = (uint32_t)c->dyn[DYN_FILT2].count;
	c->last_batch.n_moving_listed = (uint32_t)c->n_moving_listed;
	c->last_batch.general_voices = (uint32_t)c->dyn[DYN_REST].count;
	c->last_noise = a2amd_noise_batch_info{};
	c->last_noise.class_voices = (uint32_t)c->leaf[LEAF_NOISEPAN].count;
	c->last_noise.standin_voices = c->n_noise_standin;
	c->last_noise.quiet_voices = c->n_noise_quiet;
	c->last_noise_filter = a2amd_noise_filter_batch_info{};
	c->last_noise_filter.class_voices = (uint32_t)c->leaf[LEAF_NOISEFILTPAN].count;
	c->last_noise_filter.quiet_voices = c->n_noise_filt_quiet;
	c->last_noise_filter.min_voices = (uint32_t)c->sw.nzf_min;
	c->last_bare = a2amd_bare_batch_info{};
	c->last_bare.class_voices = (uint32_t)c->leaf[LEAF_OSCBARE].count;
	c->last_bare.quiet_voices = c->n_bare_quiet;
	c->last_bare.gliding_voices = c->n_bare_gliding;
	c->last_bare.record_voices = c->n_bare_records;
	c->last_bare.mono_drivers = c->n_mono_drivers;
	LeafPass lp = { pend, e1, use_win, oscpan_alone(c), false };
	const std::function<int()> mid = [&]() -> int {
		if(!c->sw.vmspec_early || !vmwin_ok || !vm_spec_wanted(c))
			return 0;
		if(int r = launch_leaves(c, lp))
			return r;
		flush_commits(c, pend);
		return vm_speculate(c);
	};
	if(use_win) {
		if(int r = issue_windows(c, c->d_dyn, c->dyn, mid))
			return r;
		if(vmwin_ok)
			if(int r = vm_predict(c))
				return r;
	}
	if(int r = launch_leaves(c, lp))
		return r;
	if(e1 && !lp.solo)
		HIPCHK(c, hipEventRecord(e1, c->stream));
	if(use_win && vmwin_ok && !c->vm.spec_launched_now && vm_spec_wanted(c)) {
		flush_commits(c, pend);
		if(int r = vm_speculate(c))
			return r;
	}
	vm_note_batch(c, use_win && vmwin_ok);
	return 0;
}

int issue_kernels(a2amd_ctx *c, unsigned phases, hipEvent_t e0, hipEvent_t e1, hipEvent_t e2)
{
	const bool has_sub = (phases & A2AMD_RENDER_SUBTREES) != 0, has_root = (phases & A2AMD_RENDER_ROOT) != 0;
	const bool consume = c->consume_ok && has_sub && has_root;
	const bool consume_sub = c->consume_ok && has_sub && !has_root;
	A2DCommitSet pend;
	pend.n = 0;
	pend.c[0].nlist = pend.c[1].nlist = 0;
	if(phases & A2AMD_RENDER_SUBTREES) {
		if(c->sub_resume < 0)
			if(int r = issue_leaf_phase(c, consume, consume_sub, e0, e1, &pend))
				return r;
		const int dstart = c->sub_resume >= 0 ? c->sub_resume : (int)c->depth_ranges.size() - 1;
		c->sub_resume = -1;
		c->paused_at = 0;
		for(int d = dstart; d >= 1; --d) {
			if(int r = launch_depth(c, d, consume ? 3 : consume_sub ? 1 : 0, &pend))
				return r;
			if((phases & A2AMD_RENDER_TAPS) && depth_has_mutes(c, d)) {
				c->paused_at = d;
				c->sub_resume = d > 1 ? d - 1 : -1;
				break;
			}
		}
		if(!(phases & A2AMD_RENDER_ROOT))
			flush_commits(c, &pend);
	}
	if(phases & A2AMD_RENDER_ROOT) {
		const bool root_stores = consume || c->consume_ok;
		if(!has_sub && !root_stores)
			HIPCHK(c, hipMemsetAsync(c->d_busmem.d, 0,
					(size_t)c->nfrags * c->cfg.channels * A2D_FRAG * sizeof(int32_t), c->stream));
		if(!c->depth_ranges.empty())
			if(int r = launch_depth(c, 0, root_stores ? 3 : 0, &pend))
				return r;
		if(!has_sub && root_stores)
			c->root_clean = true;
		flush_commits(c, &pend);
		if(e2)
			HIPCHK(c, hipEventRecord(e2, c->stream));
		c->stats.fragments += c->nfrags;
		c->stats.voice_fragments += (uint64_t)c->nfrags * (uint64_t)c->list_all.size();
	}
	return 0;
}

void drop_graphs(a2amd_ctx *c)
{
	for(int i = 0; i < 12; ++i) {
		if(c->gexec[i]) {
			hipGraphExecDestroy(c->gexec[i]);
			c->gexec[i] = nullptr;
		}
		if(c->graph[i]) {
			hipGraphDestroy(c->graph[i]);
			c->graph[i] = nullptr;
		}
	}
}

int ensure_clean(a2amd_ctx *c)
{
	if(c->consume_ok && !(c->others_clean && c->root_clean)) {
		HIPCHK(c, hipMemsetAsync(c->d_busmem.d, 0, c->bus_used * sizeof(int32_t), c->stream));
		c->others_clean = c->root_clean = true;
	}
	return 0;
}

int build_graph(a2amd_ctx *c, int slot, int steps, unsigned phases)
{
	if(c->gexec[slot]) {
		hipGraphExecDestroy(c->gexec[slot]);
		c->gexec[slot] = nullptr;
	}
	if(c->graph[slot]) {
		hipGraphDestroy(c->graph[slot]);
		c->graph[slot] = nullptr;
	}
	hipError_t e = hipStreamBeginCapture(c->stream, hipStreamCaptureModeThreadLocal);
	if(e != hipSuccess)
		return c->fail(A2AMD_EHIP, "hipStreamBeginCapture: %s", hipGetErrorString(e));
	int r = 0;
	const bool oc = c->others_clean, rc = c->root_clean;
	c->master_direct = false;
	c->capturing = true;
	for(int i = 0; i < steps && !r; ++i)
		r = issue_kernels(c, phases, nullptr, nullptr, nullptr);
	c->capturing = false;
	c->others_clean = oc;
	c->root_clean = rc;
	e = hipStreamEndCapture(c->stream, &c->graph[slot]);
	if(r)
		return r;
	if(e != hipSuccess)
		return c->fail(A2AMD_EHIP, "hipStreamEndCapture: %s", hipGetErrorString(e));
	e = hipGraphInstantiate(&c->gexec[slot], c->graph[slot], nullptr, nullptr, 0);
	if(e != hipSuccess)
		return c->fail(A2AMD_EHIP, "hipGraphInstantiate: %s", hipGetErrorString(e));
	c->gdst[slot] = c->master_dst;
	c->gdirect[slot] = c->master_direct;
	c->gconsume[slot] = c->last_bus.consume;
	return 0;
}

}
```

### audiality2_amd/csrc/a2amd_taps.h

```cpp
#pragma once
#include <hip/hip_runtime.h>
#include <stdint.h>
#include "a2amd_device.h"
#include "a2amd_dsp.h"
#include "a2amd_fm.h"

#define FAST_WPB   4
#define FAST_FCH   A2D_FAST_FCH

#define WRL(reg, val) reg = me ? (val) : reg

DEV int hermite_step(int v, unsigned ph)
{
	int p;
	asm("v_mul_i32_i24_sdwa %0, %1, %2 dst_sel:DWORD dst_unused:UNUSED_PAD src0_sel:DWORD src1_sel:BYTE_0"
			: "=v"(p) : "v"(v), "v"(ph));
	return __builtin_amdgcn_sbfe(p, 8, 17);
}

DEV int hermite4(int dm, int d0, int d1, int d2, unsigned ph)
{
	int c = (d1 - dm) >> 1;
	int a = (3 * (d0 - d1) + d2 - dm) >> 1;
	int b = dm - d0 + c - a;
	a = hermite_step(a, ph);
	a = hermite_step(a + b, ph);
	return d0 + hermite_step(a + c, ph);
}

struct __attribute__((packed, aligned(2))) Quad16 { uint32_t lo, hi; };

DEV int inter_quads(const Quad16 qa, const Quad16 qb, unsigned ph, unsigned ph2)
{
	int h0 = hermite4((int16_t)(qa.lo & 0xffff), (int)qa.lo >> 16, (int16_t)(qa.hi & 0xffff), (int)qa.hi >> 16, ph);
	int h1 = hermite4((int16_t)(qb.lo & 0xffff), (int)qb.lo >> 16, (int16_t)(qb.hi & 0xffff), (int)qb.hi >> 16, ph2);
	return h0 + h1;
}

DEV int inter_dwords(const int16_t *d, unsigned ph, unsigned dph16)
{
	const unsigned ph2 = ph + (dph16 >> 1);
	const Quad16 qa = *(const Quad16 *)(d + (int)(ph >> 8) - 1);
	const Quad16 qb = *(const Quad16 *)(d + (int)(ph2 >> 8) - 1);
	return inter_quads(qa, qb, ph, ph2);
}

typedef int Coef4 __attribute__((ext_vector_type(3)));
#define A2D_COEF_LOAD "llvm.amdgcn.struct.buffer.load.v3i32"
typedef int CoefRsrc __attribute__((ext_vector_type(4)));
extern "C" __device__ Coef4 a2d_coef_load(CoefRsrc rsrc, int vindex, int voffset, int soffset, int aux)
		__asm(A2D_COEF_LOAD);

DEV CoefRsrc coef_rsrc(const int *wavecoef)
{
	const uint64_t b = (uint64_t)wavecoef;
	CoefRsrc r;
	r.x = rfl((int)(unsigned)b);
	r.y = rfl((int)(((unsigned)(b >> 32) & 0xffffu) | ((4u * A2D_COEF_WORDS) << 16)));
	r.z = -1;
	r.w = 0x00020000;
	return r;
}

DEV int coef_base(unsigned doff) { return (int)(doff * (4u * A2D_COEF_WORDS)); }

DEV int hermite_ct(const Coef4 k, unsigned ph)
{
	int t = hermite_step(k.x, ph);
	t = hermite_step(wadd(t, k.y), ph);
	return hermite_step(wadd(t, k.z >> 16), ph);
}

DEV int inter_coefs(const Coef4 ka, unsigned pa, const Coef4 kb, unsigned pb)
{
	int d;
	asm("v_add_u32_sdwa %0, sext(%1), sext(%2) dst_sel:DWORD dst_unused:UNUSED_PAD src0_sel:WORD_0 src1_sel:WORD_0"
			: "=v"(d) : "v"(ka.z), "v"(kb.z));
	return wadd(wadd(d, hermite_ct(ka, pa)), hermite_ct(kb, pb));
}

DEV int frac_x(unsigned ph)
{
	int x;
	const int seven = 7;
	asm("v_lshlrev_b32_sdwa %0, %1, %2 dst_sel:DWORD dst_unused:UNUSED_PAD src0_sel:DWORD src1_sel:BYTE_0"
			: "=v"(x) : "v"(seven), "v"(ph));
	return x;
}

DEV int hermite_cx(const Coef4 k, unsigned ph)
{
	const int x = frac_x(ph);
	int t = wmul(k.x, x) >> 15;
	t = wmul(wadd(t, k.y), x) >> 15;
	t = wmul(wadd(t, k.z >> 16), x) >> 15;
	return wadd((int)(int16_t)(k.z & 0xffff), t);
}

DEV int inter_coefs_x(const Coef4 ka, unsigned pa, const Coef4 kb, unsigned pb)
{
	return hermite_cx(ka, pa) + hermite_cx(kb, pb);
}

DEV Coef4 coef_at(const CoefRsrc rs, int cb, unsigned ph)
{
	return a2d_coef_load(rs, (int)(ph >> 8), 0, cb, 0);
}

DEV unsigned tap_phase(uint64_t ph, unsigned ldph)
{
	const unsigned lo = (unsigned)ph & 0xffffu, hi = (unsigned)(ph >> 16);
	return hi + ((lo + ldph) >> 16);
}

DEV unsigned lane_dph(int lane, unsigned dph)
{
	unsigned t = (unsigned)lane * dph;
	asm("" : "+v"(t));
	return t;
}

DEV int64_t div_trunc_exact(int64_t n, int d)
{
	int64_t q = (int64_t)((double)n / (double)d);
	const int64_t r = n - q * d;
	if(n >= 0) {
		if(r < 0) --q; else if(r >= d) ++q;
	} else {
		if(r > 0) ++q; else if(r <= -(int64_t)d) --q;
	}
	return q;
}


template<int N>
DEV void flush_acc(int *busmem, int off, int nch, int f0, int nf, int lane, int dbg,
		int (&acc0)[N], int (&acc1)[N])
{
#pragma unroll
	for(int j = 0; j < N; ++j) {
		if(j < nf && off >= 0 && !(dbg & 1)) {
			int *dst = busmem + off + (size_t)(f0 + j) * nch * A2D_FRAG;
			if(acc0[j])
				atomicAdd(&dst[lane], acc0[j]);
			if(acc1[j])
				atomicAdd(&dst[A2D_FRAG + lane], acc1[j]);
		}
		acc0[j] = 0;
		acc1[j] = 0;
	}
}
```

### audiality2_amd/replay.py

```python
import ctypes as C
import gzip
import lzma

import numpy as np

T_FRAGMENT, T_INIT, T_DEINIT, T_WRITE, T_PROCESS, T_INLINE_END, T_WAVE, T_CONFIG, T_WAVEDROP = range(1, 10)
MIPLEVELS = 10
WAVEPRE = 1
WAVEPOST = 131


class Trace:

    def __init__(self, path):
        opener = gzip.open if str(path).endswith(".gz") else lzma.open if str(path).endswith(".xz") else open
        with opener(path, "rb") as f:
            raw = f.read()
        words = np.frombuffer(raw[: len(raw) // 4 * 4], dtype="<i4")
        self.records = []
        self.waves = {}
        self.config = None
        i = 0
        n = len(words)
        while i + 8 <= n:
            r = tuple(int(x) for x in words[i : i + 8])
            i += 8
            op = r[0]
            if op == T_WAVE:
                wid, wtype, flags, period, levels = r[1:6]
                sizes = words[i : i + MIPLEVELS].astype(np.uint32)
                i += MIPLEVELS
                data = []
                for lv in range(levels):
                    cnt = WAVEPRE + int(sizes[lv]) + WAVEPOST
                    nw = (cnt + 1) // 2
                    d = words[i : i + nw].view("<i2")[:cnt].copy()
                    i += nw
                    data.append(d)
                self.waves[wid] = dict(type=wtype, flags=flags & 0xFFFFFFFF, period=period,
                                       sizes=[int(s) for s in sizes], data=data)
                self.records.append((T_WAVE, wid, 0, 0, 0, 0, 0, 0))
            elif op == T_CONFIG:
                self.config = dict(samplerate=r[1], basepitch=r[2], channels=r[3],
                                   buffer=r[4], noiseseed=r[5] & 0xFFFFFFFF)
            else:
                self.records.append(r)
        if self.config is None:
            raise ValueError("trace without CONFIG record")
        self.kinds = {r[1]: r[3] for r in self.records if r[0] == T_INIT}

    @property
    def total_frames(self):
        return sum(r[1] for r in self.records if r[0] == T_FRAGMENT)


class a2amd_config(C.Structure):
    _fields_ = [("struct_size", C.c_uint32), ("samplerate", C.c_int32),
                ("basepitch", C.c_int32), ("channels", C.c_int32),
                ("device", C.c_int32), ("max_batch", C.c_uint32),
                ("stream", C.c_void_p)]


class a2amd_wavedesc(C.Structure):
    _fields_ = [("type", C.c_int32), ("flags", C.c_uint32), ("period", C.c_uint32),
                ("size", C.c_uint32 * MIPLEVELS),
                ("data", C.POINTER(C.c_int16) * MIPLEVELS)]


class a2amd_noise_batch_info(C.Structure):
    _fields_ = [("quiet_launched", C.c_uint32), ("quiet_voices", C.c_uint32),
                ("class_voices", C.c_uint32), ("standin_voices", C.c_uint32)]

    def __repr__(self):
        return "noise_batch_info(" + ", ".join(f"{n}={getattr(self, n)}" for n, _ in self._fields_) + ")"


class a2amd_noise_filter_batch_info(C.Structure):
    _fields_ = [("quiet_launched", C.c_uint32), ("quiet_voices", C.c_uint32),
                ("class_voices", C.c_uint32), ("min_voices", C.c_uint32)]

    def __repr__(self):
        return "noise_filter_batch_info(" + ", ".join(f"{n}={getattr(self, n)}" for n, _ in self._fields_) + ")"


class a2amd_sweep_batch_info(C.Structure):
    _fields_ = [("pass_launched", C.c_uint32), ("filters", C.c_uint32),
                ("ramp_windows", C.c_uint32), ("standin_voices", C.c_uint32)]

    def __repr__(self):
        return "sweep_batch_info(" + ", ".join(f"{n}={getattr(self, n)}" for n, _ in self._fields_) + ")"


class a2amd_bus_info(C.Structure):
    _fields_ = [(n, C.c_uint32) for n in ("driver_voices", "driver_ramping", "driver_windows_dropped", "fbd_voices",
                                          "generic_voices", "consume", "master_direct")]

    def __repr__(self):
        return "bus_info(" + ", ".join(f"{n}={getattr(self, n)}" for n, _ in self._fields_) + ")"


class a2amd_bare_batch_info(C.Structure):
    _fields_ = [(n, C.c_uint32) for n in ("launched", "class_voices", "quiet_voices", "gliding_voices", "record_voices",
                                          "vpw", "mono_drivers", "reserved")]

    def __repr__(self):
        return "bare_batch_info(" + ", ".join(f"{n}={getattr(self, n)}" for n, _ in self._fields_) + ")"


class a2amd_fbdpan_batch_info(C.Structure):
    _fields_ = [(n, C.c_uint32) for n in ("launched", "class_voices", "quiet_voices", "gliding_voices", "record_voices",
                                          "max_delays")] + [("reserved", C.c_uint32 * 2)]

    def __repr__(self):
        return "fbdpan_batch_info(" + ", ".join(f"{n}={getattr(self, n)}" for n, _ in self._fields_[:-1]) + ")"


class a2amd_bus_windows_info(C.Structure):
    _fields_ = [(n, C.c_uint32) for n in ("fbd_dropped", "fbdpan_voices", "fbdpan_gliding", "fbdpan_windows", "refused_tiling",
                                          "refused_cap", "window_cap", "launched")]

    def __repr__(self):
        return "bus_windows_info(" + ", ".join(f"{n}={getattr(self, n)}" for n, _ in self._fields_) + ")"


class a2amd_vm_batch_info(C.Structure):
    _fields_ = [("listed", C.c_uint32), ("class_voices", C.c_uint32 * 3), ("other_voices", C.c_uint32),
                ("pending", C.c_uint32), ("fused", C.c_uint32), ("not_fused", C.c_uint32),
                ("spec_valid", C.c_uint32), ("spec_taken", C.c_uint32), ("spec_miss", C.c_uint32),
                ("spec_next", C.c_uint32), ("spec_why_not", C.c_uint32), ("records", C.c_uint32),
                ("idle_known", C.c_uint32), ("idle", C.c_uint32 * 3), ("quiet_launched", C.c_uint32 * 3)]

    def __repr__(self):
        return ("vm_batch_info(" + ", ".join(f"{n}={list(getattr(self, n)) if n in ('class_voices', 'idle', 'quiet_launched') else getattr(self, n)}"
                                             for n, _ in self._fields_) + ")")


class a2amd_vm_state(C.Structure):
    _fields_ = [("waketime", C.c_uint32), ("state", C.c_uint8), ("func", C.c_uint8), ("pc", C.c_uint16),
                ("r", C.c_int32 * 64)]


class Backend:

    def __init__(self, lib, prefix, samplerate, basepitch, channels=2, device=0,
                 max_batch=64, stream=None):
        self.lib, self.prefix, self.channels = lib, prefix, channels

        def fn(name, restype, *argtypes):
            f = getattr(lib, prefix + name)
            f.restype, f.argtypes = restype, list(argtypes)
            return f

        vp, i32, u32, u64 = C.c_void_p, C.c_int, C.c_uint, C.c_uint64
        self._open = fn("open", i32, C.POINTER(a2amd_config), C.POINTER(vp))
        self._close = fn("close", None, vp)
        self._err = fn("last_error", C.c_char_p, vp)
        self._wave_upload = fn("wave_upload", i32, vp, u64, C.POINTER(a2amd_wavedesc))
        self._wave_drop = fn("wave_drop", i32, vp, u64)
        self._fragment = fn("fragment", i32, vp, u32)
        self._unit_init = fn("unit_init", i32, vp, u64, i32, u32, i32, i32, i32, i32, u32)
        self._unit_deinit = fn("unit_deinit", i32, vp, i32)
        self._unit_write = fn("unit_write", i32, vp, i32, i32, i32, u32, u32, i32)
        self._unit_process = fn("unit_process", i32, vp, i32, u32, u32, C.POINTER(C.c_uint32))
        self._inline_end = fn("inline_end", i32, vp, i32)
        self._unit_clients = fn("unit_clients", i32, vp, i32, u32)
        self._unit_inject = fn("unit_inject", i32, vp, i32, u32, u32, C.POINTER(C.POINTER(C.c_int32)))
        self._unit_tapped = fn("unit_tapped", i32, vp, i32, u32, C.POINTER(C.POINTER(C.c_int32)))
        self._render = fn("render", i32, vp, u32, C.POINTER(C.POINTER(C.c_int32)), u32)
        self._set_pt = fn("set_pitch_table", i32, vp, C.POINTER(C.c_uint32))
        self._get_pt = fn("get_pitch_table", i32, vp, C.POINTER(C.c_uint32))
        self.has_walk = hasattr(lib, prefix + "voice_process")
        if self.has_walk:
            self._voice_process = fn("voice_process", i32, vp, i32, u32, u32, C.POINTER(C.c_uint32))
            self._voice_slot = fn("voice_slot", i32, vp, i32)
            self._default_map = fn("default_map", C.POINTER(C.c_uint8), vp, C.POINTER(u32))
        self._fragment_repeat_noise = None
        if hasattr(lib, prefix + "fragment_repeat_noise"):
            self._fragment_repeat_noise = fn("fragment_repeat_noise", i32, vp, u32, u32, C.POINTER(C.c_uint32))
        self._last_batch_noise = None
        if hasattr(lib, prefix + "last_batch_noise"):
            self._last_batch_noise = fn("last_batch_noise", i32, vp, C.POINTER(a2amd_noise_batch_info))
        self._last_batch_noise_filter = None
        if hasattr(lib, prefix + "last_batch_noise_filter"):
            self._last_batch_noise_filter = fn("last_batch_noise_filter", i32, vp, C.POINTER(a2amd_noise_filter_batch_info))
        self._fragment_repeat = None
        if hasattr(lib, prefix + "fragment_repeat"):
            self._fragment_repeat = fn("fragment_repeat", i32, vp, u32, u32)
        self._last_batch_sweeps = None
        if hasattr(lib, prefix + "last_batch_sweeps"):
            self._last_batch_sweeps = fn("last_batch_sweeps", i32, vp, C.POINTER(a2amd_sweep_batch_info))
        self._last_batch_buses = None
        if hasattr(lib, prefix + "last_batch_buses"):
            self._last_batch_buses = fn("last_batch_buses", i32, vp, C.POINTER(a2amd_bus_info))
        self._last_batch_bare = None
        if hasattr(lib, prefix + "last_batch_bare"):
            self._last_batch_bare = fn("last_batch_bare", i32, vp, C.POINTER(a2amd_bare_batch_info))
        self._last_batch_fbdpan = None
        if hasattr(lib, prefix + "last_batch_fbdpan"):
            self._last_batch_fbdpan = fn("last_batch_fbdpan", i32, vp, C.POINTER(a2amd_fbdpan_batch_info))
        self._last_batch_bus_windows = None
        if hasattr(lib, prefix + "last_batch_bus_windows"):
            self._last_batch_bus_windows = fn("last_batch_bus_windows", i32, vp, C.POINTER(a2amd_bus_windows_info))
        self.has_vm = hasattr(lib, prefix + "vm_adopt")
        if self.has_vm:
            self._fragment_offset = fn("fragment_offset", i32, vp, u32)
            self._vm_program = fn("vm_program", i32, vp, u64, C.POINTER(C.c_uint32), u32)
            self._vm_adopt = fn("vm_adopt", i32, vp, i32, i32, C.POINTER(a2amd_vm_state), C.POINTER(C.c_int32),
                                C.POINTER(C.c_uint8), C.c_uint32, C.c_uint32, vp, i32)
            self._vm_expect_cuts = fn("vm_expect_cuts", i32, vp, C.POINTER(C.c_uint32), i32)
            self._vm_recall = fn("vm_recall", i32, vp, C.POINTER(C.c_int32), u32, C.POINTER(a2amd_vm_state), vp)
        self._last_batch_vm = None
        if hasattr(lib, prefix + "last_batch_vm"):
            self._last_batch_vm = fn("last_batch_vm", i32, vp, C.POINTER(a2amd_vm_batch_info))
        self.has_capture = hasattr(lib, prefix + "wave_upload_captured_post")
        if self.has_capture:
            self._capture_begin = fn("capture_begin", i32, vp)
            self._capture_end = fn("capture_end", i32, vp, C.POINTER(vp))
            self._capture_frames = fn("capture_frames", u32, vp)
            self._capture_free = fn("capture_free", None, vp)
            self._wave_upload_captured = fn("wave_upload_captured", i32, vp, u64, C.POINTER(a2amd_wavedesc), vp)
            self._wave_upload_captured_post = fn("wave_upload_captured_post", i32, vp, u64, C.POINTER(a2amd_wavedesc), vp, u32)
            self._wave_stats = fn("wave_stats", i32, vp, C.POINTER(u64), C.POINTER(u32), C.POINTER(u32))
        cfg = a2amd_config(C.sizeof(a2amd_config), samplerate, basepitch, channels,
                           device, max_batch, stream)
        self.ctx = vp()
        rc = self._open(C.byref(cfg), C.byref(self.ctx))
        if rc != 0:
            raise RuntimeError(f"{prefix}open failed: {rc} "
                               f"{self._err(None).decode(errors='replace')}")
        self.noise = C.c_uint32(0)
        self._keep = []

    def close(self):
        if self.ctx:
            self._close(self.ctx)
            self.ctx = None

    def _chk(self, rc, what):
        if rc < 0:
            msg = self._err(self.ctx)
            raise RuntimeError(f"{self.prefix}{what}: {rc} {msg.decode(errors='replace') if msg else ''}")
        return rc

    def wave_upload(self, key, wtype, flags, period, sizes, data):
        d = a2amd_wavedesc()
        d.type, d.flags, d.period = wtype, flags, period
        for lv, arr in enumerate(data):
            arr = np.ascontiguousarray(arr, dtype=np.int16)
            self._keep.append(arr)
            d.size[lv] = sizes[lv]
            d.data[lv] = arr.ctypes.data_as(C.POINTER(C.c_int16))
        return self._chk(self._wave_upload(self.ctx, key, C.byref(d)), "wave_upload")

    def capture_begin(self):
        return self._chk(self._capture_begin(self.ctx), "capture_begin")

    def capture_end(self):
        cap = C.c_void_p()
        self._chk(self._capture_end(self.ctx, C.byref(cap)), "capture_end")
        return cap if cap.value else None

    def capture_frames(self, cap):
        return self._capture_frames(cap)

    def capture_free(self, cap):
        self._capture_free(cap)

    def wave_upload_captured(self, key, wtype, flags, period, sizes, cap, chunk=None, check=True):
        d = a2amd_wavedesc()
        d.type, d.flags, d.period = wtype, flags, period
        for lv, n in enumerate(sizes):
            d.size[lv] = n
        if chunk is None:
            rc = self._wave_upload_captured(self.ctx, key, C.byref(d), cap)
        else:
            rc = self._wave_upload_captured_post(self.ctx, key, C.byref(d), cap, chunk)
        return self._chk(rc, "wave_upload_captured") if check else rc

    def wave_stats(self):
        h2d, up, res = C.c_uint64(), C.c_uint32(), C.c_uint32()
        self._chk(self._wave_stats(self.ctx, C.byref(h2d), C.byref(up), C.byref(res)), "wave_stats")
        return h2d.value, up.value, res.value

    def wave_drop(self, key):
        return self._chk(self._wave_drop(self.ctx, key), "wave_drop")

    def fragment(self, frames):
        return self._chk(self._fragment(self.ctx, frames), "fragment")

    def fragment_repeat(self, frames, count):
        if self._fragment_repeat is None:
            raise RuntimeError(f"this library has no {self.prefix}fragment_repeat")
        return self._chk(self._fragment_repeat(self.ctx, frames, count), "fragment_repeat")

    def last_batch_sweeps(self):
        if self._last_batch_sweeps is None:
            raise RuntimeError(f"this library has no {self.prefix}last_batch_sweeps")
        bi = a2amd_sweep_batch_info()
        self._chk(self._last_batch_sweeps(self.ctx, C.byref(bi)), "last_batch_sweeps")
        return bi

    def fragment_repeat_noise(self, frames, count):
        if self._fragment_repeat_noise is None:
            raise RuntimeError(f"this library has no {self.prefix}fragment_repeat_noise")
        return self._chk(self._fragment_repeat_noise(self.ctx, frames, count, C.byref(self.noise)),
                         "fragment_repeat_noise")

    def last_batch_noise(self):
        if self._last_batch_noise is None:
            raise RuntimeError(f"this library has no {self.prefix}last_batch_noise")
        bi = a2amd_noise_batch_info()
        self._chk(self._last_batch_noise(self.ctx, C.byref(bi)), "last_batch_noise")
        return bi

    def last_batch_noise_filter(self):
        if self._last_batch_noise_filter is None:
            raise RuntimeError(f"this library has no {self.prefix}last_batch_noise_filter")
        bi = a2amd_noise_filter_batch_info()
        self._chk(self._last_batch_noise_filter(self.ctx, C.byref(bi)), "last_batch_noise_filter")
        return bi

    def last_batch_buses(self):
        if self._last_batch_buses is None:
            raise RuntimeError(f"this library has no {self.prefix}last_batch_buses")
        bi = a2amd_bus_info()
        self._chk(self._last_batch_buses(self.ctx, C.byref(bi)), "last_batch_buses")
        return bi

    def last_batch_bare(self):
        if self._last_batch_bare is None:
            raise RuntimeError(f"this library has no {self.prefix}last_batch_bare")
        bi = a2amd_bare_batch_info()
        self._chk(self._last_batch_bare(self.ctx, C.byref(bi)), "last_batch_bare")
        return bi

    def last_batch_fbdpan(self):
        if self._last_batch_fbdpan is None:
            raise RuntimeError(f"this library has no {self.prefix}last_batch_fbdpan")
        bi = a2amd_fbdpan_batch_info()
        self._chk(self._last_batch_fbdpan(self.ctx, C.byref(bi)), "last_batch_fbdpan")
        return bi

    def last_batch_bus_windows(self):
        if self._last_batch_bus_windows is None:
            raise RuntimeError(f"this library has no {self.prefix}last_batch_bus_windows")
        bi = a2amd_bus_windows_info()
        self._chk(self._last_batch_bus_windows(self.ctx, C.byref(bi)), "last_batch_bus_windows")
        return bi

    def last_batch_vm(self):
        if self._last_batch_vm is None:
            raise RuntimeError(f"this library has no {self.prefix}last_batch_vm")
        bi = a2amd_vm_batch_info()
        self._chk(self._last_batch_vm(self.ctx, C.byref(bi)), "last_batch_vm")
        return bi

    def fragment_offset(self, offset):
        return self._chk(self._fragment_offset(self.ctx, offset), "fragment_offset")

    def vm_program(self, key, words):
        code = (C.c_uint32 * len(words))(*[w & 0xffffffff for w in words])
        return self._chk(self._vm_program(self.ctx, key, code, len(words)), "vm_program")

    def vm_adopt(self, head_unit, prog, state, wires, now, msdur, check=True):
        wu = (C.c_int32 * 64)(*([-1] * 64))
        wr = (C.c_uint8 * 64)()
        for r, (u, ureg) in wires.items():
            wu[r], wr[r] = u, ureg
        rc = self._vm_adopt(self.ctx, head_unit, prog, C.byref(state), wu, wr, now & 0xffffffff, msdur, None, 0)
        return self._chk(rc, "vm_adopt") if check else rc

    def vm_expect_cuts(self, when):
        arr = (C.c_uint32 * max(len(when), 1))(*[w & 0xffffffff for w in when])
        return self._chk(self._vm_expect_cuts(self.ctx, arr, len(when)), "vm_expect_cuts")

    def vm_recall(self, head_units):
        n = len(head_units)
        out = (a2amd_vm_state * n)()
        self._chk(self._vm_recall(self.ctx, (C.c_int32 * n)(*head_units), n, out, None), "vm_recall")
        return list(out)

    def last_error(self):
        msg = self._err(self.ctx)
        return msg.decode(errors="replace") if msg else ""

    def unit_init(self, voice_key, kind, flags, nin, nout, wired, transpose=0, wakefrac=0):
        return self._chk(self._unit_init(self.ctx, voice_key, kind, flags, nin, nout, wired,
                                         transpose, wakefrac), "unit_init")

    def unit_deinit(self, unit):
        return self._chk(self._unit_deinit(self.ctx, unit), "unit_deinit")

    def unit_write(self, unit, reg, value, start=0, dur=0, transpose=0):
        return self._chk(self._unit_write(self.ctx, unit, reg, value, start, dur, transpose),
                         "unit_write")

    def unit_process(self, unit, offset, frames, use_noise=True):
        return self._chk(self._unit_process(self.ctx, unit, offset, frames,
                                            C.byref(self.noise) if use_noise else None),
                         "unit_process")

    def voice_process(self, units, offset, frames):
        if self.has_walk:
            return self._chk(self._voice_process(self.ctx, units[0], offset, frames, C.byref(self.noise)),
                             "voice_process")
        for u in units:
            self.unit_process(u, offset, frames)
        return 0

    def mark_default(self, units):
        n = C.c_uint(0)
        m = self._default_map(self.ctx, C.byref(n))
        slot = self._chk(self._voice_slot(self.ctx, units[0]), "voice_slot")
        assert m and slot < n.value
        m[slot] = 1

    def inline_end(self, unit):
        return self._chk(self._inline_end(self.ctx, unit), "inline_end")

    def unit_clients(self, unit, mode):
        return self._chk(self._unit_clients(self.ctx, unit, mode), "unit_clients")

    def unit_inject(self, unit, offset, audio):
        audio = np.ascontiguousarray(audio, dtype=np.int32)
        ptrs = (C.POINTER(C.c_int32) * audio.shape[0])()
        for c in range(audio.shape[0]):
            ptrs[c] = audio[c].ctypes.data_as(C.POINTER(C.c_int32))
        return self._chk(self._unit_inject(self.ctx, unit, offset, audio.shape[1], ptrs), "unit_inject")

    def unit_tapped(self, unit, fragment):
        ptrs = (C.POINTER(C.c_int32) * 8)()
        n = self._chk(self._unit_tapped(self.ctx, unit, fragment, ptrs), "unit_tapped")
        return np.stack([np.ctypeslib.as_array(ptrs[c], shape=(64,)).copy() for c in range(n)])

    def render(self, capacity_frames, phases=15):
        out = np.zeros((self.channels, max(capacity_frames, 1)), dtype=np.int32)
        ptrs = (C.POINTER(C.c_int32) * self.channels)()
        for c in range(self.channels):
            ptrs[c] = out[c].ctypes.data_as(C.POINTER(C.c_int32))
        n = self._chk(self._render(self.ctx, phases, ptrs, capacity_frames), "render")
        return out[:, :n]

    def set_pitch_table(self, tab):
        tab = np.ascontiguousarray(tab, dtype=np.uint32)
        return self._chk(self._set_pt(self.ctx, tab.ctypes.data_as(C.POINTER(C.c_uint32))), "set_pt")

    def get_pitch_table(self):
        tab = np.zeros(128, dtype=np.uint32)
        self._chk(self._get_pt(self.ctx, tab.ctypes.data_as(C.POINTER(C.c_uint32))), "get_pt")
        return tab


def replay(trace, backend, batch=64, check_noise=True, max_fragments=None):
    umap, wmap = {}, {}
    outs = []
    nfrag = 0
    pending = 0
    backend.noise.value = trace.config["noiseseed"]
    for r in trace.records:
        op = r[0]
        if op == T_FRAGMENT:
            if max_fragments is not None and nfrag >= max_fragments:
                break
            if pending and nfrag % batch == 0:
                outs.append(backend.render(pending))
                pending = 0
            backend.fragment(r[1])
            pending += r[1]
            nfrag += 1
        elif op == T_WAVE:
            w = trace.waves[r[1]]
            wmap[r[1]] = backend.wave_upload(0x1000 + r[1], w["type"], w["flags"], w["period"],
                                             w["sizes"], w["data"])
        elif op == T_WAVEDROP:
            if pending:
                outs.append(backend.render(pending))
                pending = 0
            backend.wave_drop(0x1000 + r[1])
            wmap.pop(r[1], None)
        elif op == T_INIT:
            _, uid, voice, kind, flags, io, transpose, wakefrac = r
            umap[uid] = backend.unit_init(voice, kind, flags & 0xFFFFFFFF, io & 0xFF,
                                          (io >> 8) & 0xFF, (io >> 16) & 1, transpose, wakefrac)
        elif op == T_DEINIT:
            backend.unit_deinit(umap.pop(r[1]))
        elif op == T_WRITE:
# ... 31 lines not shown
```

### include/a2amd.h

```cpp
#ifndef A2AMD_H
#define A2AMD_H

#include <stdint.h>

#ifdef __cplusplus
extern "C" {
#endif

#define A2AMD_MAXFRAG      64
#define A2AMD_MAXCHANNELS   8
#define A2AMD_MIPLEVELS    10
#define A2AMD_WAVEPRE       1
#define A2AMD_WAVEPOST    131
#define A2AMD_MAXCHAIN     16

typedef struct a2amd_ctx a2amd_ctx;

typedef enum a2amd_errors {
	A2AMD_OK = 0,
	A2AMD_ENODEVICE   = -1,
	A2AMD_EINVAL      = -2,
	A2AMD_ENOMEM      = -3,
	A2AMD_EUNSUPPORTED= -4,
	A2AMD_ESTATE      = -5,
// ... 24 lines not shown
	A2AMD_NKINDS
} a2amd_unitkind;

#define A2AMD_PROCADD 0x00000001u

#define A2AMD_WOFF     0
#define A2AMD_WNOISE   1
#define A2AMD_WWAVE    2
#define A2AMD_WMIPWAVE 3
#define A2AMD_LOOPED   0x00000100u

typedef struct a2amd_config {
	uint32_t struct_size;
	int32_t  samplerate;
	int32_t  basepitch;
	int32_t  channels;
	int32_t  device;
	uint32_t max_batch;
	void    *stream;
} a2amd_config;

typedef struct a2amd_wavedesc {
	int32_t  type;
	uint32_t flags;
	uint32_t period;
	uint32_t size[A2AMD_MIPLEVELS];
	const int16_t *data[A2AMD_MIPLEVELS];
} a2amd_wavedesc;

int  a2amd_open(const a2amd_config *cfg, a2amd_ctx **out);
void a2amd_close(a2amd_ctx *ctx);
const char *a2amd_last_error(const a2amd_ctx *ctx);
const char *a2amd_version(void);
const char *a2amd_source_stamp(void);
int  a2amd_device_count(void);

int  a2amd_set_pitch_table(a2amd_ctx *ctx, const uint32_t *tab128);
int  a2amd_get_pitch_table(const a2amd_ctx *ctx, uint32_t *tab128);

int  a2amd_wave_upload(a2amd_ctx *ctx, uint64_t key, const a2amd_wavedesc *w);
int  a2amd_wave_drop(a2amd_ctx *ctx, uint64_t key);

typedef struct a2amd_capture a2amd_capture;
int  a2amd_capture_begin(a2amd_ctx *ctx);
int  a2amd_capture_end(a2amd_ctx *ctx, a2amd_capture **cap);
unsigned a2amd_capture_frames(const a2amd_capture *cap);
void a2amd_capture_free(a2amd_capture *cap);
int  a2amd_wave_upload_captured(a2amd_ctx *ctx, uint64_t key, const a2amd_wavedesc *w, const a2amd_capture *cap);
int  a2amd_wave_stats(a2amd_ctx *ctx, uint64_t *h2d_bytes, uint32_t *uploaded, uint32_t *resident);

int  a2amd_fragment(a2amd_ctx *ctx, unsigned frames);
int  a2amd_fragment_offset(a2amd_ctx *ctx, unsigned offset);

int  a2amd_unit_init(a2amd_ctx *ctx, uint64_t voice_key, int kind,
		unsigned flags, int ninputs, int noutputs, int wired_out,
		int transpose, unsigned wakefrac);
int  a2amd_unit_deinit(a2amd_ctx *ctx, int unit);

int  a2amd_unit_write(a2amd_ctx *ctx, int unit, int reg, int value,
		unsigned start, unsigned duration, int transpose);

int  a2amd_unit_process(a2amd_ctx *ctx, int unit, unsigned offset,
		unsigned frames, uint32_t *noisestate);
int  a2amd_voice_process(a2amd_ctx *ctx, int head_unit, unsigned offset, unsigned frames,
		uint32_t *noisestate);
int  a2amd_voice_slot(a2amd_ctx *ctx, int unit);
int  a2amd_voice_markable(a2amd_ctx *ctx, int unit);
int  a2amd_default_hold(a2amd_ctx *ctx, const uint32_t *slots, unsigned n, unsigned lo, int on);
int  a2amd_default_release_all(a2amd_ctx *ctx);
uint8_t *a2amd_default_map(a2amd_ctx *ctx, unsigned *nslots);

#define A2AMD_XIO_TAP     1u
#define A2AMD_XIO_INJECT  2u
#define A2AMD_XIO_MUTE    4u
int  a2amd_unit_clients(a2amd_ctx *ctx, int unit, unsigned mode);
int  a2amd_unit_insertable(a2amd_ctx *ctx, int unit);
int  a2amd_render_paused(a2amd_ctx *ctx);
int  a2amd_unit_insert(a2amd_ctx *ctx, int unit, unsigned fragment, unsigned offset, unsigned frames,
		const int32_t *const *bufs);
int  a2amd_unit_inject(a2amd_ctx *ctx, int unit, unsigned offset, unsigned frames,
		const int32_t *const *bufs);
int  a2amd_unit_tapped(a2amd_ctx *ctx, int unit, unsigned fragment, const int32_t **bufs);

int  a2amd_inline_end(a2amd_ctx *ctx, int unit);

#define A2AMD_RENDER_SUBTREES 1u
#define A2AMD_RENDER_ROOT     2u
#define A2AMD_RENDER_UPLOAD   4u
#define A2AMD_RENDER_READBACK 8u
#define A2AMD_RENDER_TAPS     64u
#define A2AMD_RENDER_KEEP    16u
#define A2AMD_RENDER_ASYNC   32u
#define A2AMD_RENDER_EXCHANGE 128u
#define A2AMD_RENDER_ALL     15u
int  a2amd_render(a2amd_ctx *ctx, unsigned phases, int32_t *const *out,
		unsigned out_capacity_frames);
int  a2amd_collect(a2amd_ctx *ctx, int32_t *const *out, unsigned out_capacity_frames);
int  a2amd_replay(a2amd_ctx *ctx, unsigned steps);
int  a2amd_rootbus(a2amd_ctx *ctx, void **devptr, uint64_t *bytes);
int  a2amd_rootbus_copy(a2amd_ctx *ctx, void *stage, int to_stage);

int  a2amd_dist_unique_id(void *id128);
int  a2amd_dist_init(a2amd_ctx *ctx, const void *id128, int rank, int nranks);
int  a2amd_dist_init_local(a2amd_ctx *const *ctxs, int n);
int  a2amd_render_group(a2amd_ctx *const *ctxs, int n, unsigned phases, int32_t *const *out,
		unsigned out_capacity_frames);

int  a2amd_fragment_repeat(a2amd_ctx *ctx, unsigned frames, unsigned count);


typedef struct a2amd_stats {
	uint64_t fragments;
	uint64_t voice_fragments;
	uint64_t records;
	uint64_t launches;
	double   last_kernel_ms;
	double   last_leaf_ms;
	uint32_t live_units, live_voices, live_waves, reserved;
	double   timed_leaf_ms;
	double   timed_all_ms;
	uint64_t timed_batches;
} a2amd_stats;
int  a2amd_get_stats(a2amd_ctx *ctx, a2amd_stats *st);
int  a2amd_set_profiling(a2amd_ctx *ctx, int on);
typedef struct a2amd_batch_info {
	uint32_t o2f_launched;
	uint32_t o2f_voices;
	uint32_t o2f_vpg;
	uint32_t o2f_max_vpg;
	uint32_t o2f_class;
	uint32_t o2f_listed;
	uint32_t recs_voices;
	uint32_t win_voices;
	uint32_t win_slabs;
	uint32_t n_moving_listed;
	uint32_t general_voices;
} a2amd_batch_info;
int  a2amd_last_batch(const a2amd_ctx *ctx, a2amd_batch_info *bi);

#ifdef __cplusplus
}
#endif

#include "a2amd_noise.h"
#include "a2amd_noisepan.h"
#include "a2amd_noisefilt.h"
#include "a2amd_sweep.h"
#include "a2amd_bus.h"
#include "a2amd_wavepost.h"
#include "a2amd_oscbare.h"
#include "a2amd_fbdpan.h"
#include "a2amd_buswin.h"
#include "a2amd_vmbatch.h"

#endif
```

Measured before the change: 506.9 billion voice-samples/s.

## Add voice-major super-chunk path to 2-osc pan leaf with LDS tile accumulation

Adds a voice-major loop to the 2-oscillator pan leaf kernel for super-chunks of 16 fragments whose frames are all whole. Each voice's state is loaded once per super-chunk instead of once per 4-fragment chunk, and its output is accumulated into a per-wave shared-memory tile with wavefront-scope atomics. The tile is flushed to the bus once per voice group. This cuts repeated per-voice setup and global bus atomics, at the cost of shared memory, LDS atomics and a larger kernel. Adds a batch-info query for diagnostics, and a debug bit disables the new path.

```diff
diff --git a/audiality2_amd/build.py b/audiality2_amd/build.py
--- a/audiality2_amd/build.py
+++ b/audiality2_amd/build.py
@@ -60,7 +60,7 @@
     deps = srcs + [os.path.join(csrc, "a2amd_host.h"), os.path.join(csrc, "a2amd_switches.h"), os.path.join(csrc, "a2amd_device.h"), os.path.join(csrc, "a2amd_dsp.h"),
                    os.path.join(csrc, "a2amd_fm.h"), os.path.join(csrc, "a2amd_vmcore.h"), os.path.join(csrc, "a2amd_taps.h"), os.path.join(csrc, "a2amd_winctl.h"), os.path.join(csrc, "a2amd_vmdev.h"), os.path.join(csrc, "a2amd_noisemap.h"), os.path.join(csrc, "a2amd_noisevoice.h"), os.path.join(csrc, "a2amd_settled.h"), os.path.join(csrc, "a2amd_cutsweep.h"), os.path.join(csrc, "a2amd_filt.h"), os.path.join(ROOT, "include", "a2amd.h"),
                    os.path.join(ROOT, "include", "a2amd_noise.h"), os.path.join(ROOT, "include", "a2amd_noisepan.h"), os.path.join(ROOT, "include", "a2amd_noisefilt.h"), os.path.join(ROOT, "include", "a2amd_sweep.h"), os.path.join(ROOT, "include", "a2amd_wavepost.h"),
-                   os.path.join(ROOT, "include", "a2amd_bus.h"), os.path.join(ROOT, "include", "a2amd_oscbare.h"), os.path.join(ROOT, "include", "a2amd_fbdpan.h"), os.path.join(ROOT, "include", "a2amd_buswin.h"), os.path.join(ROOT, "include", "a2amd_vmbatch.h"), os.path.join(ROOT, "include", "a2amd_vm.h")]
+                   os.path.join(ROOT, "include", "a2amd_bus.h"), os.path.join(ROOT, "include", "a2amd_oscbare.h"), os.path.join(ROOT, "include", "a2amd_fbdpan.h"), os.path.join(ROOT, "include", "a2amd_buswin.h"), os.path.join(ROOT, "include", "a2amd_vmbatch.h"), os.path.join(ROOT, "include", "a2amd_osc2.h"), os.path.join(ROOT, "include", "a2amd_vm.h")]
     out = os.path.join(HERE, "liba2amd.so")
     flags = ["--offload-arch=gfx950", "-O3", "-std=c++17", "-fPIC", "-shared", "-Wno-unused-value"]
     want = source_hash(deps, flags)
@@ -73,7 +73,7 @@
     src = os.path.join(HERE, "csrc", "a2amd_units.c")
     deps = [src, os.path.join(ROOT, "include", "a2amd.h"), os.path.join(ROOT, "include", "a2amd_noise.h"), os.path.join(ROOT, "include", "a2amd_noisepan.h"),
             os.path.join(ROOT, "include", "a2amd_noisefilt.h"), os.path.join(ROOT, "include", "a2amd_sweep.h"), os.path.join(ROOT, "include", "a2amd_bus.h"),
-            os.path.join(ROOT, "include", "a2amd_wavepost.h"), os.path.join(ROOT, "include", "a2amd_oscbare.h"), os.path.join(ROOT, "include", "a2amd_fbdpan.h"), os.path.join(ROOT, "include", "a2amd_buswin.h"), os.path.join(ROOT, "include", "a2amd_vmbatch.h"), os.path.join(ROOT, "include", "a2amd_plugin.h"),
+            os.path.join(ROOT, "include", "a2amd_wavepost.h"), os.path.join(ROOT, "include", "a2amd_oscbare.h"), os.path.join(ROOT, "include", "a2amd_fbdpan.h"), os.path.join(ROOT, "include", "a2amd_buswin.h"), os.path.join(ROOT, "include", "a2amd_vmbatch.h"), os.path.join(ROOT, "include", "a2amd_osc2.h"), os.path.join(ROOT, "include", "a2amd_plugin.h"),
             os.path.join(ROOT, "include", "a2amd_walk.h"), os.path.join(ROOT, "include", "a2amd_vm.h")]
     out = os.path.join(HERE, "liba2amd_units.so")
     flags = ["-O2", "-Wall", "-fPIC", "-shared"]
diff --git a/audiality2_amd/csrc/a2amd_device.h b/audiality2_amd/csrc/a2amd_device.h
--- a/audiality2_amd/csrc/a2amd_device.h
+++ b/audiality2_amd/csrc/a2amd_device.h
@@ -159,6 +159,7 @@
 
 #define A2D_FAST_FCH 8
 #define A2D_OSC2_FCH 4
+#define A2D_OSC2_SCH 16
 #define A2D_MAXVPW   32
 
 struct A2DParams {
@@ -190,6 +191,25 @@
 	uint8_t         fragframes[A2D_MAXBATCH];
 	uint16_t        fragstart[A2D_MAXBATCH];
 };
+
+#ifdef __HIPCC__
+#define A2D_HD static inline __host__ __device__
+#else
+#define A2D_HD static inline
+#endif
+A2D_HD bool a2d_osc2_slice(int nfrags, int ysplit, int slice, int *c_lo, int *c_hi, int *nslices)
+{
+	const int nchunks = (nfrags + A2D_OSC2_FCH - 1) / A2D_OSC2_FCH;
+	const int per = (nchunks + ysplit - 1) / ysplit;
+	*c_lo = slice * per;
+	*c_hi = *c_lo + per < nchunks ? *c_lo + per : nchunks;
+	*nslices = (nchunks + per - 1) / per;
+	return *c_lo < nchunks;
+}
+A2D_HD bool a2d_osc2_whole(unsigned start_first, unsigned start_last, unsigned frames_last, int n)
+{
+	return start_last + frames_last - start_first == (unsigned)n * A2D_FRAG;
+}
 
 #ifdef __HIPCC__
 static inline __host__ __device__ bool a2d_noise_seed(const A2DParams &p, int f, int ui, unsigned *seed)
@@ -294,7 +314,7 @@
 		int vpw, void *stream);
 int a2d_launch_scatter_runs(const int *didx, const A2DRun *dval, int n, A2DRun *druns, void *stream);
 int a2d_launch_leaf_osc2pan(const A2DParams *dparams, const A2DParams &hp, const int *dlist, int nlist,
-		int vpw, int ysplit, int *ustage, unsigned char *staged, void *stream, A2DCommit *defer);
+		int vpw, int ysplit, int *ustage, unsigned char *staged, void *stream, A2DCommit *defer, int voice_major, int *ysplit_used);
 struct A2Switches;
 int a2d_launch_leaf_recs(const A2Switches &sw, const A2DParams *dparams, const A2DParams &hp, int nosc, int filt, const int *dlist,
 		int nlist, int vpw, void *stream, int skip_empty = 0);
diff --git a/audiality2_amd/csrc/a2amd_fast.hip b/audiality2_amd/csrc/a2amd_fast.hip
--- a/audiality2_amd/csrc/a2amd_fast.hip
+++ b/audiality2_amd/csrc/a2amd_fast.hip
@@ -574,6 +574,8 @@
 }
 
 #define OSC2_FCH A2D_OSC2_FCH
+#define OSC2_SCH A2D_OSC2_SCH
+static_assert(OSC2_SCH % OSC2_FCH == 0, "a super-chunk is whole chunks");
 enum { OV_MODE = 0, OV_WAVE, OV_DPHASE, OV_PHLO, OV_PHHI, OV_PRAMP, OV_P = 6, OV_A = 10, OV_NWORDS = 14 };
 enum { OD_MM = 0, OD_DPH, OD_SIZEM, OD_DOFF, OD_NWORDS };
 
@@ -606,13 +608,87 @@
 	WRL(so[OV_A + 2], o.a.delta); WRL(so[OV_A + 3], o.a.timer);
 }
 
+struct Osc2Voice {
+	unsigned dph[2], sizem[2];
+	int cb[2], amp[2];
+	uint64_t ph[2], end[2];
+};
+
+template<bool WHOLE>
+DEV void osc2_chunk(const CoefRsrc &crs, Osc2Voice &s, const unsigned (&ldph)[2], const int (&nfr)[OSC2_FCH],
+		const unsigned (&pre)[OSC2_FCH], int nf, bool park, int (&xs)[OSC2_FCH])
+{
+	Coef4 ka[2][OSC2_FCH], kb[2][OSC2_FCH];
+	unsigned pa[2][OSC2_FCH], pb[2][OSC2_FCH];
+#pragma unroll
+	for(int o = 0; o < 2; ++o) {
+		const unsigned dph = s.dph[o], sizem = s.sizem[o];
+		uint64_t ph = s.ph[o];
+		uint64_t phs[OSC2_FCH];
+		if(!(sizem & (sizem - 1)) && !(ph >> 48)) {
+			const uint64_t mask = ((uint64_t)sizem << 24) - 1;
+#pragma unroll
+			for(int j = 0; j < OSC2_FCH; ++j)
+				phs[j] = (ph + (uint64_t)dph * (WHOLE ? (unsigned)(j * A2D_FRAG) : pre[j])) & mask;
+			ph = phs[OSC2_FCH - 1] + (uint64_t)dph * (WHOLE ? (unsigned)A2D_FRAG : (unsigned)nfr[OSC2_FCH - 1]);
+		} else {
+#pragma unroll
+			for(int j = 0; j < OSC2_FCH; ++j) {
+				ph = wrap_phase(ph, sizem);
+				phs[j] = ph;
+				ph += (uint64_t)dph * (WHOLE ? (unsigned)A2D_FRAG : (unsigned)nfr[j]);
+			}
+		}
+#pragma unroll
+		for(int j = 0; j < OSC2_FCH; ++j) {
+			pa[o][j] = tap_phase(phs[j], ldph[o]);
+			asm("" : "+v"(pa[o][j]));
+			pb[o][j] = pa[o][j] + (dph >> 17);
+			ka[o][j] = coef_at(crs, s.cb[o], pa[o][j]);
+			kb[o][j] = coef_at(crs, s.cb[o], pb[o][j]);
+		}
+		if(park) {
+			uint64_t e = ph;
+#pragma unroll
+			for(int j = OSC2_FCH - 2; j >= 0; --j)
+				if(nf == j + 1)
+					e = phs[j] + (uint64_t)dph * (WHOLE ? (unsigned)A2D_FRAG : (unsigned)nfr[j]);
+			s.end[o] = e;
+		}
+		s.ph[o] = ph;
+	}
+#pragma unroll
+	for(int o = 0; o < 2; ++o)
+#pragma unroll
+		for(int j = 0; j < OSC2_FCH; ++j) {
+			const int y = mul64s(inter_coefs(ka[o][j], pa[o][j], kb[o][j], pb[o][j]), s.amp[o], 17);
+			xs[j] = o ? wadd(xs[j], y) : y;
+		}
+}
+
+DEV void osc2_voice_from_lanes(Osc2Voice &s, unsigned (&ldph)[2], unsigned (&mm)[2], const int (&od)[2][OD_NWORDS],
+		const int (&amp_l)[2], const int (&phlo_l)[2], const int (&phhi_l)[2], int v, unsigned before, int lane)
+{
+#pragma unroll
+	for(int o = 0; o < 2; ++o) {
+		mm[o] = (unsigned)rdl(od[o][OD_MM], v);
+		s.dph[o] = (unsigned)rdl(od[o][OD_DPH], v);
+		s.sizem[o] = (unsigned)rdl(od[o][OD_SIZEM], v);
+		s.cb[o] = coef_base((unsigned)rdl(od[o][OD_DOFF], v));
+		s.amp[o] = rdl(amp_l[o], v);
+		const uint64_t phase = (uint64_t)(unsigned)rdl(phlo_l[o], v) | ((uint64_t)(unsigned)rdl(phhi_l[o], v) << 32);
+		s.ph[o] = (phase >> mm[o]) + (uint64_t)before * s.dph[o];
+		ldph[o] = lane_dph(lane, s.dph[o]);
+	}
+}
+
 #define OSC2_WPE 4
 __global__ __launch_bounds__(64 * FAST_WPB) __attribute__((amdgpu_waves_per_eu(OSC2_WPE, OSC2_WPE)))
 void k_leaf_osc2pan(const A2DParams *__restrict__ pp, const int *__restrict__ list, int nlist, int vpw,
 		int ysplit, const A2DVoice *__restrict__ voices, const int *ustate, int *ustage,
 		const int16_t *__restrict__ wavepool, const A2DWave *__restrict__ waves,
 		const uint32_t *__restrict__ ptab, int *__restrict__ busmem, const int *__restrict__ wavecoef,
-		unsigned char *__restrict__ staged)
+		unsigned char *__restrict__ staged, int vmajor)
 {
 	const A2DParams &p = *pp;
 	const int wv = rfl((int)(threadIdx.x >> 6));
@@ -626,14 +702,11 @@
 	FastPtrs g = { wavepool, waves, ptab, dbg };
 	const CoefRsrc crs = coef_rsrc(wavecoef);
 
-	const int nchunks = (nfrags + OSC2_FCH - 1) / OSC2_FCH;
-	const int per = (nchunks + ysplit - 1) / ysplit;
 	const int slice = blockIdx.y;
-	const int c_lo = slice * per, c_hi = min(nchunks, c_lo + per);
-	const bool last_slice = c_hi >= nchunks;
-	if(c_lo >= nchunks)
+	int c_lo, c_hi, nslices;
+	if(!a2d_osc2_slice(nfrags, ysplit, slice, &c_lo, &c_hi, &nslices))
 		return;
-	const int nslices = (nchunks + per - 1) / per;
+	const bool last_slice = c_hi * OSC2_FCH >= nfrags;
 
 	int ffr[A2D_MAXBATCH / 64], fst[A2D_MAXBATCH / 64];
 #pragma unroll
@@ -687,95 +760,108 @@
 	}
 	const unsigned long long unsettled_mask = __ballot(mine && !settled_l);
 
-	for(int c = c_lo; c < c_hi; ++c) {
-		const int f0 = c * OSC2_FCH;
-		const int nf = min((int)OSC2_FCH, nfrags - f0);
-		int acc0[OSC2_FCH], acc1[OSC2_FCH], nfr[OSC2_FCH];
-#pragma unroll
-		for(int j = 0; j < OSC2_FCH; ++j) {
-			acc0[j] = acc1[j] = 0;
-			nfr[j] = (j < nf) ? frames_of(ffr, f0 + j) : 0;
-		}
-		const unsigned before = (unsigned)frames_of(fst, f0);
-		unsigned pre[OSC2_FCH];
-		pre[0] = 0;
-#pragma unroll
-		for(int j = 1; j < OSC2_FCH; ++j)
-			pre[j] = pre[j - 1] + (unsigned)nfr[j - 1];
-		int cur_off = rdl(my_off, 0), cur_nch = rdl(my_nch, 0);
-		for(int v = 0; v < nv; ++v) {
-			if(!rdl(settled_l, v))
-				continue;
-			const int voff = rdl(my_off, v);
-			if(voff != cur_off) {
-				flush_acc(busmem, cur_off, cur_nch, f0, nf, lane, dbg, acc0, acc1);
-				cur_off = voff;
-				cur_nch = rdl(my_nch, v);
-			}
-			const int v0 = rdl(v0l, v), v1 = rdl(v1l, v);
-			int xs[OSC2_FCH];
-			uint64_t endph[2];
-			Coef4 ka[2][OSC2_FCH], kb[2][OSC2_FCH];
-			unsigned pa[2][OSC2_FCH], pb[2][OSC2_FCH];
-			int amps[2];
-#pragma unroll
-			for(int o = 0; o < 2; ++o) {
-				const unsigned mm = (unsigned)rdl(od[o][OD_MM], v), dph = (unsigned)rdl(od[o][OD_DPH], v);
-				const unsigned sizem = (unsigned)rdl(od[o][OD_SIZEM], v), doff = (unsigned)rdl(od[o][OD_DOFF], v);
-				amps[o] = rdl(amp_l[o], v);
-				const uint64_t phase = (uint64_t)(unsigned)rdl(phlo_l[o], v) |
-						((uint64_t)(unsigned)rdl(phhi_l[o], v) << 32);
-				uint64_t ph = (phase >> mm) + (uint64_t)before * dph;
-				const unsigned ldph = lane_dph(lane, dph);
-				const int cb = coef_base(doff);
-				uint64_t phs[OSC2_FCH];
-				if(!(sizem & (sizem - 1)) && !(ph >> 48)) {
-					const uint64_t mask = ((uint64_t)sizem << 24) - 1;
-#pragma unroll
-					for(int j = 0; j < OSC2_FCH; ++j)
-						phs[j] = (ph + (uint64_t)dph * pre[j]) & mask;
-					ph = phs[OSC2_FCH - 1] + (uint64_t)dph * (unsigned)nfr[OSC2_FCH - 1];
-				} else {
+	__shared__ int tiles[FAST_WPB][OSC2_SCH][2][A2D_FRAG];
+	int (*const tile)[2][A2D_FRAG] = tiles[wv];
+	if(vmajor)
+#pragma unroll
+		for(int r = 0; r < OSC2_SCH; ++r)
+			tile[r][0][lane] = tile[r][1][lane] = 0;
+	for(int s_lo = c_lo; s_lo < c_hi; s_lo += OSC2_SCH / OSC2_FCH) {
+		const int s_hi = min(c_hi, s_lo + OSC2_SCH / OSC2_FCH);
+		const int fa = s_lo * OSC2_FCH, nfs = min(nfrags, s_hi * OSC2_FCH) - fa;
+		const bool last = last_slice && s_hi == c_hi;
+		const unsigned before = (unsigned)frames_of(fst, fa);
+		if(vmajor && a2d_osc2_whole(before, (unsigned)frames_of(fst, fa + nfs - 1), (unsigned)frames_of(ffr, fa + nfs - 1), nfs)) {
+			const int nsc = s_hi - s_lo;
+			const int nopre_i[OSC2_FCH] = { 0, 0, 0, 0 };
+			const unsigned nopre_u[OSC2_FCH] = { 0, 0, 0, 0 };
+			int cur_off = rdl(my_off, 0), cur_nch = rdl(my_nch, 0);
+			for(int v = 0; v < nv; ++v) {
+				if(!rdl(settled_l, v))
+					continue;
+				const int voff = rdl(my_off, v);
+				if(voff != cur_off) {
+					flush_tile(busmem, cur_off, cur_nch, fa, nfs, nsc * OSC2_FCH, lane, dbg, tile);
+					cur_off = voff;
+					cur_nch = rdl(my_nch, v);
+				}
+				const int v0 = rdl(v0l, v), v1 = rdl(v1l, v);
+				Osc2Voice s;
+				unsigned ldph[2], mm[2];
+				osc2_voice_from_lanes(s, ldph, mm, od, amp_l, phlo_l, phhi_l, v, before, lane);
+				for(int k = 0; k < nsc; ++k) {
+					const bool park = last && k == nsc - 1;
+					int xs[OSC2_FCH];
+					osc2_chunk<true>(crs, s, ldph, nopre_i, nopre_u, nfs - k * OSC2_FCH, park, xs);
 #pragma unroll
 					for(int j = 0; j < OSC2_FCH; ++j) {
-						ph = wrap_phase(ph, sizem);
-						phs[j] = ph;
-						ph += (uint64_t)dph * (unsigned)nfr[j];
+						tile_add(&tile[k * OSC2_FCH + j][0][lane], mul64s(xs[j], v0, 24));
+						tile_add(&tile[k * OSC2_FCH + j][1][lane], mul64s(xs[j], v1, 24));
 					}
-				}
+					if(park) {
+						const bool me = lane == v;
+#pragma unroll
+						for(int o = 0; o < 2; ++o) {
+							const uint64_t endph = s.end[o] << mm[o];
+							WRL(phlo_l[o], (int)(unsigned)endph);
+							WRL(phhi_l[o], (int)(unsigned)(endph >> 32));
+						}
+					}
+				}
+			}
+			flush_tile(busmem, cur_off, cur_nch, fa, nfs, nsc * OSC2_FCH, lane, dbg, tile);
+			continue;
+		}
+		for(int c = s_lo; c < s_hi; ++c) {
+			const int f0 = c * OSC2_FCH;
+			const int nf = min((int)OSC2_FCH, nfrags - f0);
+			int acc0[OSC2_FCH], acc1[OSC2_FCH], nfr[OSC2_FCH];
+#pragma unroll
+			for(int j = 0; j < OSC2_FCH; ++j) {
+				acc0[j] = acc1[j] = 0;
+				nfr[j] = (j < nf) ? frames_of(ffr, f0 + j) : 0;
+			}
+			const unsigned before = (unsigned)frames_of(fst, f0);
+			unsigned pre[OSC2_FCH];
+			pre[0] = 0;
+#pragma unroll
+			for(int j = 1; j < OSC2_FCH; ++j)
+				pre[j] = pre[j - 1] + (unsigned)nfr[j - 1];
+			const bool park = last && c == s_hi - 1;
+			int cur_off = rdl(my_off, 0), cur_nch = rdl(my_nch, 0);
+			for(int v = 0; v < nv; ++v) {
+				if(!rdl(settled_l, v))
+					continue;
+				const int voff = rdl(my_off, v);
+				if(voff != cur_off) {
+					flush_acc(busmem, cur_off, cur_nch, f0, nf, lane, dbg, acc0, acc1);
+					cur_off = voff;
+					cur_nch = rdl(my_nch, v);
+				}
+				const int v0 = rdl(v0l, v), v1 = rdl(v1l, v);
+				Osc2Voice s;
+				unsigned ldph[2], mm[2];
+				int xs[OSC2_FCH];
+				osc2_voice_from_lanes(s, ldph, mm, od, amp_l, phlo_l, phhi_l, v, before, lane);
+				osc2_chunk<false>(crs, s, ldph, nfr, pre, nf, park, xs);
 #pragma unroll
 				for(int j = 0; j < OSC2_FCH; ++j) {
-					pa[o][j] = tap_phase(phs[j], ldph);
-					asm("" : "+v"(pa[o][j]));
-					pb[o][j] = pa[o][j] + (dph >> 17);
-					ka[o][j] = coef_at(crs, cb, pa[o][j]);
-					kb[o][j] = coef_at(crs, cb, pb[o][j]);
-				}
-				endph[o] = ph << mm;
-			}
-#pragma unroll
-			for(int o = 0; o < 2; ++o)
-#pragma unroll
-				for(int j = 0; j < OSC2_FCH; ++j) {
-					const int y = mul64s(inter_coefs(ka[o][j], pa[o][j], kb[o][j], pb[o][j]), amps[o], 17);
-					xs[j] = o ? wadd(xs[j], y) : y;
-				}
-#pragma unroll
-			for(int j = 0; j < OSC2_FCH; ++j) {
-				const int x = (lane < nfr[j]) ? xs[j] : 0;
-				acc0[j] = wadd(acc0[j], mul64s(x, v0, 24));
-				acc1[j] = wadd(acc1[j], mul64s(x, v1, 24));
-			}
-			if(last_slice && c == c_hi - 1) {
-				const bool me = lane == v;
-#pragma unroll
-				for(int o = 0; o < 2; ++o) {
-					WRL(phlo_l[o], (int)(unsigned)endph[o]);
-					WRL(phhi_l[o], (int)(unsigned)(endph[o] >> 32));
-				}
-			}
-		}
-		flush_acc(busmem, cur_off, cur_nch, f0, nf, lane, dbg, acc0, acc1);
+					const int x = (lane < nfr[j]) ? xs[j] : 0;
+					acc0[j] = wadd(acc0[j], mul64s(x, v0, 24));
+					acc1[j] = wadd(acc1[j], mul64s(x, v1, 24));
+				}
+				if(park) {
+					const bool me = lane == v;
+#pragma unroll
+					for(int o = 0; o < 2; ++o) {
+						const uint64_t endph = s.end[o] << mm[o];
+						WRL(phlo_l[o], (int)(unsigned)endph);
+						WRL(phhi_l[o], (int)(unsigned)(endph >> 32));
+					}
+				}
+			}
+			flush_acc(busmem, cur_off, cur_nch, f0, nf, lane, dbg, acc0, acc1);
+		}
 	}
 
 	const unsigned long long todo_mask = unsettled_mask & __ballot(lane % nslices == slice);
@@ -2722,18 +2808,20 @@
 }
 
 int a2d_launch_leaf_osc2pan(const A2DParams *dparams, const A2DParams &hp, const int *dlist, int nlist,
-		int vpw, int ysplit, int *ustage, unsigned char *staged, void *stream, A2DCommit *defer)
+		int vpw, int ysplit, int *ustage, unsigned char *staged, void *stream, A2DCommit *defer, int voice_major, int *ysplit_used)
 {
 	if(nlist <= 0)
 		return 0;
 	vpw = vpw < 1 ? 1 : (vpw > 64 ? 64 : vpw);
 	if(ysplit < 1 || !ustage || !staged)
 		ysplit = 1;
+	if(ysplit_used)
+		*ysplit_used = ysplit;
 	int nwaves = (nlist + vpw - 1) / vpw;
 	int nblocks = (nwaves + FAST_WPB - 1) / FAST_WPB;
 	hipLaunchKernelGGL(k_leaf_osc2pan, dim3(nblocks, ysplit), dim3(64 * FAST_WPB), 0, (hipStream_t)stream,
 			dparams, dlist, nlist, vpw, ysplit, hp.voices, (const int *)hp.ustate,
-			ysplit > 1 ? ustage : hp.ustate, hp.wavepool, hp.waves, hp.ptab, hp.busmem, hp.wavecoef, staged);
+			ysplit > 1 ? ustage : hp.ustate, hp.wavepool, hp.waves, hp.ptab, hp.busmem, hp.wavecoef, staged, voice_major);
 	if(ysplit > 1) {
 		A2DCommit cm = { dlist, nlist, 2, ustage, staged };
 		if(defer)
diff --git a/audiality2_amd/csrc/a2amd_host.h b/audiality2_amd/csrc/a2amd_host.h
--- a/audiality2_amd/csrc/a2amd_host.h
+++ b/audiality2_amd/csrc/a2amd_host.h
@@ -407,6 +407,7 @@
 	a2amd_noise_filter_batch_info last_noise_filter = {};
 	uint32_t n_bare_quiet = 0, n_bare_gliding = 0, n_bare_records = 0, n_mono_drivers = 0;
 	a2amd_bare_batch_info last_bare = {};
+	a2amd_osc2_batch_info last_osc2 = {};
 	a2amd_fbdpan_batch_info last_fbdpan = {};
 	a2amd_bus_windows_info last_buswin = {};
 	a2amd_bus_info last_bus = {};
diff --git a/audiality2_amd/csrc/a2amd_render.cpp b/audiality2_amd/csrc/a2amd_render.cpp
--- a/audiality2_amd/csrc/a2amd_render.cpp
+++ b/audiality2_amd/csrc/a2amd_render.cpp
@@ -464,6 +464,38 @@
 	return A2AMD_OK;
 }
 
+int a2amd_last_batch_osc2(const a2amd_ctx *c, a2amd_osc2_batch_info *out)
+{
+	if(!c || !out)
+		return A2AMD_EINVAL;
+	*out = c->last_osc2;
+	if(!out->launched || c->blob_nfrags < 1 || c->blob_nfrags > A2D_MAXBATCH)
+		return A2AMD_OK;
+	unsigned start[A2D_MAXBATCH];
+	for(int f = 0, acc = 0; f < c->blob_nfrags; ++f) {
+		start[f] = (unsigned)acc;
+		acc += (int)c->blob_frames[f];
+	}
+	unsigned n = 0;
+	for(int slice = 0; slice < (int)out->ysplit; ++slice) {
+		int c_lo, c_hi, nslices;
+		if(!a2d_osc2_slice(c->blob_nfrags, (int)out->ysplit, slice, &c_lo, &c_hi, &nslices))
+			break;
+		for(int s_lo = c_lo; s_lo < c_hi; s_lo += A2D_OSC2_SCH / A2D_OSC2_FCH, ++n) {
+			const int s_hi = std::min(c_hi, s_lo + A2D_OSC2_SCH / A2D_OSC2_FCH);
+			const int fa = s_lo * A2D_OSC2_FCH, fb = std::min(c->blob_nfrags, s_hi * A2D_OSC2_FCH);
+			if(out->voice_major && a2d_osc2_whole(start[fa], start[fb - 1], c->blob_frames[fb - 1], fb - fa))
+				++out->superchunks_voice_major;
+			else {
+				++out->superchunks_chunk_major;
+				if(n < 64)
+					out->chunk_major_mask |= 1ull << n;
+			}
+		}
+	}
+	return A2AMD_OK;
+}
+
 int a2amd_last_batch_fbdpan(const a2amd_ctx *c, a2amd_fbdpan_batch_info *out)
 {
 	if(!c || !out)
diff --git a/audiality2_amd/csrc/a2amd_sched.cpp b/audiality2_amd/csrc/a2amd_sched.cpp
--- a/audiality2_amd/csrc/a2amd_sched.cpp
+++ b/audiality2_amd/csrc/a2amd_sched.cpp
@@ -1545,9 +1545,15 @@
 	else if(osc2pan.count) {
 		int vpw, ysplit;
 		pick_fast_shape(c->sw, osc2pan.count, c->nfrags * A2D_FAST_FCH / A2D_OSC2_FCH, &vpw, &ysplit, 16);
+		const int voice_major = !(c->sw.debug & 16);
 		if(a2d_launch_leaf_osc2pan(c->d_params, c->hparams, list + osc2pan.first, osc2pan.count,
-				vpw, ysplit, c->d_ustage.d, c->d_staged.d + osc2pan.first, c->stream, &pend.c[pend.n]))
+				vpw, ysplit, c->d_ustage.d, c->d_staged.d + osc2pan.first, c->stream, &pend.c[pend.n], voice_major, &ysplit))
 			return c->fail(A2AMD_EHIP, "2-osc leaf launch failed: %s", hipGetErrorString(hipGetLastError()));
+		c->last_osc2.launched = 1;
+		c->last_osc2.voices = (uint32_t)osc2pan.count;
+		c->last_osc2.vpw = (uint32_t)std::min(std::max(vpw, 1), 64);
+		c->last_osc2.ysplit = (uint32_t)ysplit;
+		c->last_osc2.voice_major = (uint32_t)voice_major;
 		if(pend.c[pend.n].nlist)
 			++pend.n;
 		++c->stats.launches;
@@ -1682,6 +1688,7 @@
 	c->last_bare.gliding_voices = c->n_bare_gliding;
 	c->last_bare.record_voices = c->n_bare_records;
 	c->last_bare.mono_drivers = c->n_mono_drivers;
+	c->last_osc2 = a2amd_osc2_batch_info{};
 	LeafPass lp = { pend, e1, use_win, oscpan_alone(c), false };
 	const std::function<int()> mid = [&]() -> int {
 		if(!c->sw.vmspec_early || !vmwin_ok || !vm_spec_wanted(c))
diff --git a/audiality2_amd/csrc/a2amd_taps.h b/audiality2_amd/csrc/a2amd_taps.h
--- a/audiality2_amd/csrc/a2amd_taps.h
+++ b/audiality2_amd/csrc/a2amd_taps.h
@@ -150,3 +150,24 @@
 		acc1[j] = 0;
 	}
 }
+
+DEV void tile_add(int *w, int x)
+{
+	(void)__hip_atomic_fetch_add(w, x, __ATOMIC_RELAXED, __HIP_MEMORY_SCOPE_WAVEFRONT);
+}
+
+DEV void flush_tile(int *busmem, int off, int nch, int f0, int nf, int nrows, int lane, int dbg, int (*tile)[2][A2D_FRAG])
+{
+	for(int r = 0; r < nrows; ++r) {
+		const int a0 = tile[r][0][lane], a1 = tile[r][1][lane];
+		tile[r][0][lane] = 0;
+		tile[r][1][lane] = 0;
+		if(r < nf && off >= 0 && !(dbg & 1)) {
+			int *dst = busmem + off + (size_t)(f0 + r) * nch * A2D_FRAG;
+			if(a0)
+				atomicAdd(&dst[lane], a0);
+			if(a1)
+				atomicAdd(&dst[A2D_FRAG + lane], a1);
+		}
+	}
+}
diff --git a/audiality2_amd/replay.py b/audiality2_amd/replay.py
--- a/audiality2_amd/replay.py
+++ b/audiality2_amd/replay.py
@@ -105,6 +105,14 @@
 
     def __repr__(self):
         return "bare_batch_info(" + ", ".join(f"{n}={getattr(self, n)}" for n, _ in self._fields_) + ")"
+
+
+class a2amd_osc2_batch_info(C.Structure):
+    _fields_ = [(n, C.c_uint32) for n in ("launched", "voices", "vpw", "ysplit", "voice_major", "superchunks_voice_major",
+                                          "superchunks_chunk_major", "reserved")] + [("chunk_major_mask", C.c_uint64)]
+
+    def __repr__(self):
+        return "osc2_batch_info(" + ", ".join(f"{n}={getattr(self, n)}" for n, _ in self._fields_) + ")"
 
 
 class a2amd_fbdpan_batch_info(C.Structure):
@@ -195,6 +203,9 @@
         self._last_batch_bare = None
         if hasattr(lib, prefix + "last_batch_bare"):
             self._last_batch_bare = fn("last_batch_bare", i32, vp, C.POINTER(a2amd_bare_batch_info))
+        self._last_batch_osc2 = None
+        if hasattr(lib, prefix + "last_batch_osc2"):
+            self._last_batch_osc2 = fn("last_batch_osc2", i32, vp, C.POINTER(a2amd_osc2_batch_info))
         self._last_batch_fbdpan = None
         if hasattr(lib, prefix + "last_batch_fbdpan"):
             self._last_batch_fbdpan = fn("last_batch_fbdpan", i32, vp, C.POINTER(a2amd_fbdpan_batch_info))
@@ -332,6 +343,13 @@
             raise RuntimeError(f"this library has no {self.prefix}last_batch_bare")
         bi = a2amd_bare_batch_info()
         self._chk(self._last_batch_bare(self.ctx, C.byref(bi)), "last_batch_bare")
+        return bi
+
+    def last_batch_osc2(self):
+        if self._last_batch_osc2 is None:
+            raise RuntimeError(f"this library has no {self.prefix}last_batch_osc2")
+        bi = a2amd_osc2_batch_info()
+        self._chk(self._last_batch_osc2(self.ctx, C.byref(bi)), "last_batch_osc2")
         return bi
 
     def last_batch_fbdpan(self):
diff --git a/include/a2amd.h b/include/a2amd.h
--- a/include/a2amd.h
+++ b/include/a2amd.h
@@ -200,5 +200,6 @@
 #include "a2amd_fbdpan.h"
 #include "a2amd_buswin.h"
 #include "a2amd_vmbatch.h"
+#include "a2amd_osc2.h"
 
 #endif
diff --git a/include/a2amd_osc2.h b/include/a2amd_osc2.h
--- /dev/null
+++ b/include/a2amd_osc2.h
@@ -0,0 +1,27 @@
+#ifndef A2AMD_OSC2_H
+#define A2AMD_OSC2_H
+#include <stdint.h>
+
+#ifdef __cplusplus
+extern "C" {
+#endif
+
+struct a2amd_ctx;
+
+typedef struct a2amd_osc2_batch_info {
+	uint32_t launched;
+	uint32_t voices;
+	uint32_t vpw;
+	uint32_t ysplit;
+	uint32_t voice_major;
+	uint32_t superchunks_voice_major;
+	uint32_t superchunks_chunk_major;
+	uint32_t reserved;
+	uint64_t chunk_major_mask;
+} a2amd_osc2_batch_info;
+int a2amd_last_batch_osc2(const struct a2amd_ctx *ctx, a2amd_osc2_batch_info *out);
+
+#ifdef __cplusplus
+}
+#endif
+#endif
```

After: 525.8 billion voice-samples/s (median of 6 runs). 3.7% higher.
